# martinResearch/PySparseLP

Measured on AMD Instinct MI355X. Metric: admm_iterations_per_sec, higher is better.
Workload: dtype f64

## Files before the change

include/slp_hip_ext.h:

```cpp
#ifndef SLP_HIP_EXT_H
#define SLP_HIP_EXT_H

#include <stdint.h>

#include "slp_hip.h"
#include "slp_hip_ext_admm_batch.h"
#include "slp_hip_ext_dga_batch.h"

#ifdef __cplusplus
extern "C" {
#endif

int slp_cp_batch_set_stop_gap(slp_cp_batch *s, double tol_gap, double tol_feas, int64_t check_every);
int slp_cp_batch_gap_state(slp_cp_batch *s, int64_t *iterations, int32_t *stopped, double *primal, double *bound, double *violation);

#ifdef __cplusplus
}
#endif
#endif
```

pysparselp_amd/_lib.py:

```python
import ctypes
import os

import numpy as np

_HERE = os.path.dirname(os.path.abspath(__file__))
_VARIANT = os.environ.get("SLP_LIB_VARIANT")
LIB_PATH = os.path.join(_HERE, f"libslp_hip_{_VARIANT}.so" if _VARIANT else "libslp_hip.so")

ORDER_AUTO, ORDER_SEQUENTIAL, ORDER_TREE = 0, 1, 2

_lib = None
_device = None

c_i64 = ctypes.c_int64
c_int = ctypes.c_int
c_dbl = ctypes.c_double
c_vp = ctypes.c_void_p

_SIGNATURES = {
    "slp_version": (c_int, []),
    "slp_build_flags": (c_int, []),
    "slp_device_count": (c_int, []),
    "slp_init": (c_int, [c_int]),
    "slp_synchronize": (c_int, []),
    "slp_trim": (c_int, []),
    "slp_cached_bytes": (c_i64, []),
    "slp_alloc_stats": (c_int, [c_vp, c_int]),
    "slp_last_error": (ctypes.c_char_p, []),
    "slp_timer_start": (c_int, []),
    "slp_timer_stop": (c_int, [c_vp]),
    "slp_matrix_create": (c_vp, [c_i64, c_i64, c_vp, c_vp, c_vp]),
    "slp_matrix_create_stacked": (c_vp, [c_i64, c_i64, c_vp, c_vp, c_vp, c_i64, c_vp, c_vp, c_vp]),
    "slp_matrix_destroy": (None, [c_vp]),
    "slp_matrix_nnz": (c_i64, [c_vp]),
    "slp_matrix_spmv": (c_int, [c_vp, c_vp, c_vp, c_int]),
    "slp_matrix_spmv_t": (c_int, [c_vp, c_vp, c_vp, c_int]),
    "slp_matrix_spmv_abs_pow": (c_int, [c_vp, c_int, c_dbl, c_vp, c_vp]),
    "slp_matrix_spmv2": (c_int, [c_vp, c_int, c_vp, c_vp, c_vp, c_vp]),
    "slp_matrix_download": (c_int, [c_vp, c_int, c_vp, c_vp, c_vp]),
    "slp_matrix_download_rows": (c_int, [c_vp, c_int, c_i64, c_i64, c_vp, c_vp, c_vp]),
    "slp_matrix_bench_spmv": (c_int, [c_vp, c_int, c_int, c_int, c_vp]),
    "slp_product_timing": (c_int, [c_int]),
    "slp_product_timing_read": (c_int, [c_vp]),
    "slp_matrix_gather_rows": (c_vp, [c_vp, c_i64, c_vp, c_vp]),
    "slp_matrix_spmv_kernel": (c_int, [c_vp, c_int]),
    "slp_matrix_set_format": (c_int, [c_vp, c_int]),
    "slp_matrix_release_csr": (c_int, [c_vp]),
    "slp_device_memory": (c_int, [c_vp, c_vp]),
    "slp_matrix_normal": (c_vp, [c_vp, c_dbl, c_dbl]),
    "slp_matrix_remove_columns": (c_vp, [c_vp, c_vp, c_vp, c_vp]),
    "slp_matrix_format_bytes": (c_i64, [c_vp, c_int]),
    "slp_matrix_chunked_create": (c_vp, [c_i64]),
    "slp_matrix_chunked_append": (c_int, [c_vp, c_vp]),
    "slp_matrix_chunks": (c_i64, [c_vp]),
    "slp_matrix_product_launches": (c_i64, [c_vp, c_int]),
    "slp_matrix_strip_width": (c_i64, [c_vp, c_int]),
    "slp_matrix_tall_rows": (c_i64, [c_vp, c_int]),
    "slp_matrix_chunked_expect": (c_int, [c_vp, c_i64]),
    "slp_matrix_chunked_expect_rows": (c_int, [c_vp, c_i64, c_i64]),
    "slp_cp_create": (c_vp, [c_i64, c_i64, c_i64, c_vp, c_vp, c_vp, c_vp, c_vp, c_vp, c_vp, c_vp, c_dbl, c_dbl, c_int]),
    "slp_cp_create_on": (c_vp, [c_vp, c_i64, c_vp, c_vp, c_vp, c_vp, c_vp, c_dbl, c_dbl, c_int]),
    "slp_cp_destroy": (None, [c_vp]),
    "slp_cp_iterate": (c_int, [c_vp, c_i64]),
    "slp_cp_primal_step": (c_int, [c_vp]),
    "slp_cp_split_form": (c_int, [c_vp]),
    "slp_cp_dual_step": (c_int, [c_vp]),
    "slp_cp_report": (c_int, [c_vp, c_vp]),
    "slp_cp_get_x": (c_int, [c_vp, c_vp]),
    "slp_cp_get_y": (c_int, [c_vp, c_vp]),
    "slp_cp_get_preconditioners": (c_int, [c_vp, c_vp, c_vp]),
    "slp_cp_bench": (c_int, [c_vp, c_i64, c_vp]),
    "slp_cp_batch_create": (c_vp, [c_i64, c_i64, c_i64, c_vp, c_vp, c_vp, c_i64, c_vp, c_int, c_vp, c_vp, c_int, c_vp, c_int, c_vp, c_int,
                                   c_dbl, c_dbl]),
    "slp_cp_batch_destroy": (None, [c_vp]),
    "slp_cp_batch_iterate": (c_int, [c_vp, c_i64]),
    "slp_cp_batch_primal_step": (c_int, [c_vp]),
    "slp_cp_batch_dual_step": (c_int, [c_vp]),
    "slp_cp_batch_report": (c_int, [c_vp, c_vp]),
    "slp_cp_batch_get_x": (c_int, [c_vp, c_vp]),
    "slp_cp_batch_get_y": (c_int, [c_vp, c_vp]),
    "slp_cp_batch_get_preconditioners": (c_int, [c_vp, c_vp, c_vp]),
    "slp_cp_batch_bench": (c_int, [c_vp, c_i64, c_vp]),
    "slp_cp_many_create": (c_vp, [c_i64, c_vp, c_vp, c_vp, c_vp, c_vp, c_vp, c_vp, c_vp, c_vp, c_vp, c_vp, c_dbl, c_dbl]),
    "slp_cp_many_destroy": (None, [c_vp]),
    "slp_cp_many_iterate": (c_int, [c_vp, c_i64]),
    "slp_cp_many_primal_step": (c_int, [c_vp]),
    "slp_cp_many_dual_step": (c_int, [c_vp]),
    "slp_cp_many_report": (c_int, [c_vp, c_vp]),
    "slp_cp_many_get_x": (c_int, [c_vp, c_vp]),
    "slp_cp_many_get_y": (c_int, [c_vp, c_vp]),
    "slp_cp_many_get_preconditioners": (c_int, [c_vp, c_vp, c_vp]),
    "slp_cp_many_form": (c_int, [c_vp, c_i64]),
    "slp_cp_many_lds_limit": (c_i64, []),
    "slp_cp_many_bench": (c_int, [c_vp, c_i64, c_vp]),
    "slp_many_cp_set_stop": (c_int, [c_vp, c_dbl, c_i64]),
    "slp_many_cp_stop_state": (c_int, [c_vp, c_vp, c_vp, c_vp]),
    "slp_many_cpgap_set_stop": (c_int, [c_vp, c_dbl, c_dbl, c_i64]),
    "slp_many_cpgap_state": (c_int, [c_vp] * 6),
    "slp_gs_create": (c_vp, [c_i64, c_vp, c_vp, c_vp]),
    "slp_gs_destroy": (None, [c_vp]),
    "slp_gs_num_levels": (c_i64, [c_vp]),
    "slp_gs_sweep_kind": (c_int, [c_vp]),
    "slp_gs_num_bands": (c_int, [c_vp]),
    "slp_gs_solve": (c_int, [c_vp, c_vp, c_vp, c_vp, c_vp, c_int, c_dbl]),
    "slp_admm_create": (c_vp, [c_i64, c_i64, c_vp, c_vp, c_vp, c_vp, c_vp, c_vp, c_vp, c_vp, c_vp, c_vp, c_vp, c_dbl, c_dbl, c_int]),
    "slp_admm_create_lp": (c_vp, [c_i64, c_i64, c_vp, c_vp, c_vp, c_vp, c_i64, c_vp, c_vp, c_vp, c_vp, c_vp, c_vp, c_vp, c_vp, c_vp, c_dbl, c_dbl,
                                  c_int, c_int]),
    "slp_matrix_precondition_rows": (c_vp, [c_vp, c_vp, c_vp]),
    "slp_matrix_standard_form": (c_vp, [c_vp, c_vp]),
    "slp_admm_destroy": (None, [c_vp]),
    "slp_admm_set_xstep": (c_int, [c_vp, c_int]),
    "slp_admm_iterate": (c_int, [c_vp, c_i64]),
    "slp_admm_sweep_step": (c_int, [c_vp]),
    "slp_admm_multiplier_step": (c_int, [c_vp]),
    "slp_admm_report": (c_int, [c_vp, c_vp]),
    "slp_admm_get_x": (c_int, [c_vp, c_vp, c_i64]),
    "slp_admm_get_lambda": (c_int, [c_vp, c_vp]),
    "slp_admm_num_levels": (c_i64, [c_vp]),
    "slp_admm_num_bands": (c_int, [c_vp]),
    "slp_admm_bench": (c_int, [c_vp, c_i64, c_vp]),
    "slp_admm_batch_create_lp": (c_vp, [c_i64, c_i64, c_vp, c_vp, c_vp, c_vp, c_i64, c_vp, c_vp, c_vp, c_vp, c_vp, c_i64, c_vp, c_int, c_vp, c_int,
                                        c_vp, c_int, c_vp, c_int, c_dbl, c_dbl, c_int]),
    "slp_admm_batch_destroy": (None, [c_vp]),
    "slp_admm_batch_iterate": (c_int, [c_vp, c_i64]),
    "slp_admm_batch_sweep_step": (c_int, [c_vp]),
    "slp_admm_batch_multiplier_step": (c_int, [c_vp]),
    "slp_admm_batch_report": (c_int, [c_vp, c_vp]),
    "slp_admm_batch_get_x": (c_int, [c_vp, c_vp, c_i64]),
    "slp_admm_batch_get_lambda": (c_int, [c_vp, c_vp]),
    "slp_admm_batch_num_levels": (c_i64, [c_vp]),
    "slp_admm_batch_form": (c_int, [c_vp]),
    "slp_admm_batch_bench": (c_int, [c_vp, c_i64, c_vp]),
    "slp_admm_many_create": (c_vp, [c_i64, c_vp, c_vp, c_vp, c_vp, c_vp, c_vp, c_vp, c_vp, c_vp, c_vp, c_vp, c_vp, c_vp, c_vp, c_vp, c_vp,
                                    c_dbl, c_dbl, c_int]),
    "slp_admm_many_destroy": (None, [c_vp]),
    "slp_admm_many_iterate": (c_int, [c_vp, c_i64]),
    "slp_admm_many_sweep_step": (c_int, [c_vp]),
    "slp_admm_many_multiplier_step": (c_int, [c_vp]),
    "slp_admm_many_report": (c_int, [c_vp, c_vp]),
    "slp_admm_many_get_x": (c_int, [c_vp, c_vp, c_int]),
    "slp_admm_many_get_lambda": (c_int, [c_vp, c_vp]),
    "slp_admm_many_num_levels": (c_i64, [c_vp, c_i64]),
    "slp_admm_many_form": (c_int, [c_vp, c_i64]),
    "slp_admm_many_lds_limit": (c_i64, []),
    "slp_admm_many_kmax": (c_i64, [c_vp, c_int]),
    "slp_admm_many_bench": (c_int, [c_vp, c_i64, c_vp]),
    "slp_many_admm_set_stop": (c_int, [c_vp, c_dbl, c_dbl, c_i64]),
    "slp_many_admm_stop_state": (c_int, [c_vp, c_vp, c_vp, c_vp, c_vp]),
    "slp_admm_cg_create": (c_vp, [c_i64, c_i64, c_vp, c_vp, c_vp, c_vp, c_vp, c_vp, c_vp, c_vp, c_dbl, c_dbl, c_int]),
    "slp_admm_cg_create_on": (c_vp, [c_vp, c_vp, c_vp, c_vp, c_vp, c_dbl, c_dbl, c_int]),
    "slp_admm_cg_create_on_mixed": (c_vp, [c_vp, c_i64, c_vp, c_vp, c_vp, c_vp, c_dbl, c_dbl, c_int]),
    "slp_blocks_create": (c_vp, [c_i64, c_i64, c_i64, c_vp, c_vp, c_vp, c_vp, c_vp, c_vp, c_vp, c_vp, c_vp, c_vp, c_vp, c_dbl]),
    "slp_blocks_create_on": (c_vp, [c_vp, c_i64, c_vp, c_vp, c_vp, c_vp, c_vp, c_dbl]),
    "slp_blocks_group_link": (c_int, [c_vp, c_int]),
    "slp_blocks_group_iterate": (c_int, [c_vp, c_int, c_i64]),
    "slp_blocks_destroy": (None, [c_vp]),
    "slp_blocks_projection_residual": (c_int, [c_vp, c_vp]),
    "slp_blocks_set_cg": (c_int, [c_vp, c_dbl, c_int]),
    "slp_blocks_set_precond": (c_int, [c_vp, c_int]),
    "slp_blocks_iterate": (c_int, [c_vp, c_i64]),
    "slp_blocks_report": (c_int, [c_vp, c_vp]),
    "slp_blocks_cg_steps": (c_i64, [c_vp]),
    "slp_blocks_get_xp": (c_int, [c_vp, c_vp, c_i64]),
    "slp_admm2_create_on": (c_vp, [c_vp, c_i64, c_vp, c_vp, c_vp, c_vp, c_vp, c_vp, c_dbl]),
    "slp_admm2_destroy": (None, [c_vp]),
    "slp_admm2_set_cg": (c_int, [c_vp, c_dbl, c_int]),
    "slp_admm2_iterate": (c_int, [c_vp, c_i64]),
    "slp_admm2_report": (c_int, [c_vp, c_vp]),
    "slp_admm2_cg_steps": (c_i64, [c_vp]),
    "slp_admm2_get_x": (c_int, [c_vp, c_vp, c_i64]),
    "slp_admm2_projection_residual": (c_int, [c_vp, c_vp]),
    "slp_dga_create_on": (c_vp, [c_vp, c_i64, c_vp, c_vp, c_vp, c_vp, c_vp]),
    "slp_dga_destroy": (None, [c_vp]),
    "slp_dga_set_path": (c_int, [c_vp, c_int]),
    "slp_dga_path": (c_int, [c_vp]),
    "slp_dga_iterate": (c_int, [c_vp, c_i64]),
    "slp_dga_iterations": (c_i64, [c_vp]),
    "slp_dga_push_random": (c_int, [c_vp, c_vp, c_i64]),
    "slp_dga_status": (c_int, [c_vp, c_vp]),
    "slp_dga_get_x": (c_int, [c_vp, c_vp]),
    "slp_dga_get_y": (c_int, [c_vp, c_vp]),
    "slp_dga_report": (c_int, [c_vp, c_vp]),
    "slp_dga_timing": (c_int, [c_vp, c_int]),
    "slp_dga_timing_read": (c_int, [c_vp, c_vp]),
    "slp_dga_line_search": (c_int, [c_vp, c_vp, c_vp, c_vp, c_vp, c_vp, c_int, c_vp, c_i64, c_vp]),
    "slp_batch_dga_create_on": (c_vp, [c_vp, c_i64, c_vp, c_i64, c_vp, c_vp, c_int, c_vp, c_int, c_vp, c_int]),
    "slp_batch_dga_destroy": (None, [c_vp]),
    "slp_batch_dga_set_path": (c_int, [c_vp, c_int]),
    "slp_batch_dga_path": (c_int, [c_vp]),
    "slp_batch_dga_sort": (c_int, [c_vp]),
    "slp_batch_dga_iterate": (c_int, [c_vp, c_i64]),
    "slp_batch_dga_iterations": (c_i64, [c_vp]),
    "slp_batch_dga_push_random": (c_int, [c_vp, c_vp, c_i64]),
    "slp_batch_dga_status": (c_int, [c_vp, c_vp]),
    "slp_batch_dga_frozen": (c_int, [c_vp, c_vp]),
    "slp_batch_dga_get_x": (c_int, [c_vp, c_vp]),
    "slp_batch_dga_get_y": (c_int, [c_vp, c_vp]),
    "slp_batch_dga_report": (c_int, [c_vp, c_vp]),
    "slp_batch_dga_timing": (c_int, [c_vp, c_int]),
    "slp_batch_dga_timing_read": (c_int, [c_vp, c_vp]),
    "slp_many_dga_create": (c_vp, [c_i64, c_vp, c_vp, c_vp, c_vp, c_vp, c_vp, c_vp, c_vp, c_vp, c_vp, c_vp, c_vp]),
    "slp_many_dga_destroy": (None, [c_vp]),
    "slp_many_dga_iterate": (c_int, [c_vp, c_i64]),
    "slp_many_dga_push_random": (c_int, [c_vp, c_vp, c_i64]),
    "slp_many_dga_status": (c_int, [c_vp, c_vp]),
    "slp_many_dga_frozen": (c_int, [c_vp, c_vp]),
    "slp_many_dga_get_x": (c_int, [c_vp, c_vp]),
    "slp_many_dga_get_y": (c_int, [c_vp, c_vp]),
    "slp_many_dga_report": (c_int, [c_vp, c_vp]),
    "slp_many_dga_timing": (c_int, [c_vp, c_int]),
    "slp_many_dga_timing_read": (c_int, [c_vp, c_vp]),
    "slp_many_dga_kmax": (c_i64, [c_vp]),
    "slp_many_dual_set_stop": (c_int, [c_vp, c_dbl, c_i64]),
    "slp_many_dual_stop_state": (c_int, [c_vp, c_vp, c_vp, c_vp]),
    "slp_admm_cg_create_on_two_sided": (c_vp, [c_vp, c_i64, c_vp, c_vp, c_vp, c_vp, c_vp, c_dbl, c_dbl, c_int]),
    "slp_admm_cg_create_on_lp": (c_vp, [c_vp, c_i64, c_vp, c_vp, c_vp, c_vp, c_vp, c_vp, c_dbl, c_dbl, c_int, c_int]),
    "slp_admm_cg_create_lp": (c_vp, [c_i64, c_i64, c_vp, c_vp, c_vp, c_vp, c_i64, c_vp, c_vp, c_vp, c_vp, c_vp, c_vp, c_vp, c_vp, c_vp,
                                     c_dbl, c_dbl, c_int, c_int]),
    "slp_admm_cg_destroy": (None, [c_vp]),
    "slp_admm_cg_set_reuse": (c_int, [c_vp, c_int]),
    "slp_admm_cg_iterate": (c_int, [c_vp, c_i64]),
    "slp_admm_cg_xstep": (c_int, [c_vp]),
    "slp_admm_cg_multiplier_step": (c_int, [c_vp]),
    "slp_admm_cg_report": (c_int, [c_vp, c_vp]),
    "slp_admm_cg_get_x": (c_int, [c_vp, c_vp, c_i64]),
    "slp_matrix_random": (c_vp, [c_i64, c_i64, c_dbl, ctypes.c_uint64, c_i64]),
    "slp_random_lp_vectors": (c_int, [c_vp, c_dbl, ctypes.c_uint64, c_i64, c_vp, c_vp, c_vp, c_vp, c_vp]),
    "slp_random_lp_vectors_eq": (c_int, [c_vp, c_dbl, ctypes.c_uint64, c_i64, c_i64, c_vp, c_vp, c_vp, c_vp, c_vp]),
    "slp_comm_unique_id": (c_int, [c_vp]),
    "slp_comm_init": (c_int, [c_int, c_int, c_vp]),
    "slp_comm_init_host": (c_int, [c_int, c_int, c_vp, c_vp]),
    "slp_comm_finalize": (c_int, []),
    "slp_comm_allreduce_host": (c_int, [c_vp, c_i64, c_int]),
    "slp_comm_barrier": (c_int, []),
    "slp_comm_bench_allreduce": (c_int, [c_i64, c_int, c_vp]),
    "slp_comm_info": (c_int, [c_vp, c_vp]),
    "slp_comm_collectives": (ctypes.c_longlong, []),
    "slp_comm_timing": (c_int, [c_int]),
    "slp_comm_timing_read": (c_int, [c_vp]),
}

EXPORTED_SYMBOLS = tuple(_SIGNATURES)

_EXT_SIGNATURES = {
    "slp_cp_batch_set_stop_gap": (c_int, [c_vp, c_dbl, c_dbl, c_i64]),
    "slp_cp_batch_gap_state": (c_int, [c_vp] * 6),
}

EXT_SYMBOLS = tuple(_EXT_SIGNATURES)

_EXT_ADMM_BATCH_SIGNATURES = {
    "slp_admm_batch_set_stop": (c_int, [c_vp, c_dbl, c_dbl, c_i64]),
    "slp_admm_batch_stop_state": (c_int, [c_vp] * 5),
}

EXT_ADMM_BATCH_SYMBOLS = tuple(_EXT_ADMM_BATCH_SIGNATURES)

_EXT_DGA_BATCH_SIGNATURES = {
    "slp_batch_dga_set_stop": (c_int, [c_vp, c_dbl, c_vp, c_i64]),
    "slp_batch_dga_stop_state": (c_int, [c_vp] * 5),
}

EXT_DGA_BATCH_SYMBOLS = tuple(_EXT_DGA_BATCH_SIGNATURES)

HOST_ALLREDUCE_FN = ctypes.CFUNCTYPE(c_int, ctypes.POINTER(c_dbl), c_i64, c_int, c_vp)


class SlpError(RuntimeError):
    """Raised for every failure reported by libslp_hip.so (and when it is absent)."""


def load():
    global _lib
    if _lib is not None:
        return _lib
    if not os.path.exists(LIB_PATH):
        raise SlpError(
            f"{LIB_PATH} is missing: build it with `python -c 'import __graft_entry__ as g; g.build()'` "
            "or `make -C pysparselp_amd/csrc`.  pysparselp_amd has no CPU fallback."
        )
    try:
        lib = ctypes.CDLL(LIB_PATH, mode=ctypes.RTLD_GLOBAL)
    except OSError as e:
        raise SlpError(f"cannot load {LIB_PATH}: {e}") from e
    for name, (res, args) in (list(_SIGNATURES.items()) + list(_EXT_SIGNATURES.items()) + list(_EXT_ADMM_BATCH_SIGNATURES.items())
                              + list(_EXT_DGA_BATCH_SIGNATURES.items())):
        fn = getattr(lib, name)
        fn.restype = res
        fn.argtypes = args
    flags = int(lib.slp_build_flags())
    if flags and not _VARIANT:
        raise SlpError(f"{LIB_PATH} is a kernel-lab build (slp_build_flags() = {flags}: bit 0 = -DSLP_ABLATION kernels with parts removed, "
                       "WRONG results; bit 1 = `make variant`): it is only loaded when SLP_LIB_VARIANT names it.  Rebuild with "
                       "`make -C pysparselp_amd/csrc clean all`.")
    _lib = lib
    return lib


def last_error():
    msg = load().slp_last_error()
    return msg.decode("utf-8", "replace") if msg else "unknown error"


def check(rc):
    if rc != 0:
        raise SlpError(last_error())


def check_handle(h):
    if not h:
        raise SlpError(last_error())
    return h


def lib(device=None):
    global _device
    l = load()
    if _device is None:
        dev = device
        if dev is None:
            dev = int(os.environ.get("SLP_DEVICE", os.environ.get("LOCAL_RANK", "0")))
            n = l.slp_device_count()
            if n > 0 and dev >= n:
                raise SlpError(f"device index {dev} (SLP_DEVICE / LOCAL_RANK) but only {n} HIP device(s) are visible")
        check(l.slp_init(int(dev)))
        _device = int(dev)
    elif device is not None and int(device) != _device:
        raise SlpError(f"process already bound to device {_device}")
    return l


def ptr(a):
    if a is None:
        return None
    assert a.flags.c_contiguous
    return a.ctypes.data_as(c_vp)


def f64(a):
    return np.ascontiguousarray(a, dtype=np.float64)


def csr_arrays(a):
    return (np.ascontiguousarray(a.indptr, dtype=np.int64), np.ascontiguousarray(a.indices, dtype=np.int32),
            np.ascontiguousarray(a.data, dtype=np.float64))
```

pysparselp_amd/csrc/slp_chunked.hip:

```cpp
#include "slp_common.h"
#include "slp_kernels.h"

slp_matrix::~slp_matrix() {
    for (slp_matrix *c : chunks) delete c;
}

namespace slp {

void composite_of_chunks(const slp_matrix *g, bool transposed, size_t k0, size_t k1, StripJds &f) {
    f.parts.clear();
    f.part_off.clear();
    f.parts_cols = transposed;
    f.ok = k1 > k0;
    f.nrow = transposed ? g->a.ncol : g->a.nrow;
    f.ncol = transposed ? g->a.nrow : g->a.ncol;
    f.nnz = 0;
    f.D = 0;
    f.tall = true;
    bool first = true;
    for (size_t k = k0; k < k1; ++k) {
        const StripJds *p = transposed ? &g->chunks[k]->fat : &g->chunks[k]->fa;
        f.parts.push_back(p);
        f.part_off.push_back(g->chunk_row0[k]);
        f.nnz += g->chunks[k]->a.nnz;
        f.D = first ? p->D : (p->D > 0 && f.D > 0 ? std::max(f.D, p->D) : 0);
        f.tall = f.tall && p->tall;
        first = false;
    }
    f.fused = f.tall && tall_fuse(f);
}

static void refresh_composites(slp_matrix *g) {
    for (int t = 0; t < 2; ++t) composite_of_chunks(g, t != 0, 0, g->chunks.size(), t ? g->fat : g->fa);
    g->at.nrow = g->a.ncol;
    g->at.ncol = g->a.nrow;
    g->at.nnz = g->a.nnz;
}

}

using namespace slp;

extern "C" {

slp_matrix *slp_matrix_chunked_create(int64_t ncol) {
    SLP_API_PTR({
        SLP_REQUIRE(ncol > 0 && ncol < ((i64)1 << 31), "slp_matrix_chunked_create: bad column count");
        ctx();
        auto *g = new slp_matrix();
        g->a.ncol = ncol;
        g->tried_fa = g->tried_fat = true;
        g->have_at = true;
        g->csr_released = true;
        return g;
    })
}

int slp_matrix_chunked_append(slp_matrix *g, slp_matrix *c) {
    SLP_API_INT({
        SLP_REQUIRE(g && c && g != c, "slp_matrix_chunked_append: NULL argument");
        SLP_REQUIRE(g->csr_released && g->a.ptr.p == nullptr && (g->a.nrow == 0 || !g->chunks.empty()),
                    "slp_matrix_chunked_append: the first argument is not a chunked matrix (slp_matrix_chunked_create)");
        SLP_REQUIRE(c->chunks.empty() && !c->csr_released, "slp_matrix_chunked_append: the chunk must be a plain matrix with its CSR");
        SLP_REQUIRE(c->a.ncol == g->a.ncol, "slp_matrix_chunked_append: the chunk has another column count");
        SLP_REQUIRE(c->a.nrow > 0 && c->a.nnz > 0, "slp_matrix_chunked_append: empty chunk");
        SLP_REQUIRE(g->borrowers == 0, "slp_matrix_chunked_append: a solver created on the chunked matrix is alive");
        SLP_REQUIRE(c->borrowers == 0 && !c->scaled, "slp_matrix_chunked_append: the chunk is in use by a solver (or was scaled in place)");
        SLP_REQUIRE(g->a.nrow % 2 == 0, "slp_matrix_chunked_append: every chunk but the last must have an even number of rows");
        Phase ph("slp_matrix_chunked_append");
        if (g->expect_rows > 0 && g->a.nrow + c->a.nrow <= g->expect_rows && !c->tried_fa) {
            const char *e = getenv("SLP_TALL_FUSE");
            if (!(e && e[0] == '0')) {
                c->tall_rows_before = g->a.nrow;
                c->tall_rows_total = g->expect_rows;
            }
        } else if (g->expect_chunks > 1 && !c->tried_fa) {
            const char *e = getenv("SLP_TALL_FUSE");
            if (!(e && e[0] == '0')) {
                i64 a = ctx().num_cu, b = g->expect_chunks;
                while (b) { const i64 t = a % b; a = b; b = t; }
                c->tall_block_multiple = ctx().num_cu / a;
            }
        }
        if (!c->tried_fa && !c->tried_fat)
            for (int t = 0; t < 2; ++t) c->tall_carry[t] = g->tall_carry[t];
        const StripJds *f0 = fast_format(c, false), *f1 = fast_format(c, true);
        SLP_REQUIRE(f0 && f1, "slp_matrix_chunked_append: the chunk does not qualify for strip copies in both orientations (too small or "
                              "unsorted rows): use an ordinary matrix for problems of that size");
        if (f0->D > 0 && f1->D > 0) {
            c->rowsq.alloc(2 * (size_t)c->a.nrow);
            matrix_row_squares(c->a, c->rowsq.p);
        }
        if (g->chunks.empty())
            for (int t = 0; t < 2; ++t) {
                const StripJds *f = t ? f1 : f0;
                if (f->tall && f->S == 1) {
                    g->tall_carry[t].C = f->C; g->tall_carry[t].dcap = f->D > 0 ? f->tall_dcap : -1;
                    g->tall_carry[t].R = f->tall_R; g->tall_carry[t].total = f->tall_total;
                }
            }
        if (f0->tall) g->tall_carry[0].blocks += f0->B;
        SLP_REQUIRE(slp_matrix_release_csr(c) == 0, slp_last_error());
        c->a.ptr.release();
        c->at.ptr.release();
        g->chunks.push_back(c);
        g->chunk_row0.push_back(g->a.nrow);
        g->a.nrow += c->a.nrow;
        g->a.nnz += c->a.nnz;
        g->a.max_row_len = std::max(g->a.max_row_len, c->a.max_row_len);
        refresh_composites(g);
        if ((i64)g->chunks.size() < g->expect_chunks) {
            std::vector<size_t> sizes;
            for (const StripJds *f : {f0, f1})
                if (f->tall)
                    for (const auto &b : f->tall_pay) sizes.push_back(b.cap);
            dev_reserve_async(sizes);
        }
    })
}

int slp_matrix_chunked_expect(slp_matrix *g, int64_t chunks) {
    SLP_API_INT({
        SLP_REQUIRE(g && g->csr_released && g->a.ptr.p == nullptr && chunks >= 0, "slp_matrix_chunked_expect: bad arguments");
        g->expect_chunks = chunks;
    })
}

int slp_matrix_chunked_expect_rows(slp_matrix *g, int64_t chunks, int64_t rows) {
    SLP_API_INT({
        SLP_REQUIRE(g && g->csr_released && g->a.ptr.p == nullptr && chunks >= 0 && rows >= 0, "slp_matrix_chunked_expect_rows: bad arguments");
        g->expect_chunks = chunks;
        g->expect_rows = rows;
    })
}

int64_t slp_matrix_chunks(const slp_matrix *g) { return g ? (int64_t)g->chunks.size() : -1; }

int64_t slp_matrix_strip_width(slp_matrix *m, int transposed) {
    if (!m) return -1;
    int64_t c = 0;
    const int rc = [&]() -> int {
        SLP_API_INT({
            const StripJds *f = fast_format(m, transposed != 0);
            if (f && !m->chunks.empty() && !f->parts.empty()) f = f->parts[0];
            c = (f && f->ok) ? (int64_t)f->C : 0;
        })
    }();
    return rc == 0 ? c : -1;
}

int64_t slp_matrix_tall_rows(slp_matrix *m, int transposed) {
    if (!m) return -1;
    int64_t r = 0;
    const int rc = [&]() -> int {
        SLP_API_INT({
            const StripJds *f = fast_format(m, transposed != 0);
            if (f && !m->chunks.empty() && !f->parts.empty()) f = f->parts[0];
            r = (f && f->ok && f->tall) ? (int64_t)f->tall_R : 0;
        })
    }();
    return rc == 0 ? r : -1;
}

int64_t slp_matrix_product_launches(const slp_matrix *g, int transposed) {
    if (!g) return -1;
    if (g->chunks.empty()) return 1;
    return (transposed ? g->fat : g->fa).fused ? 1 : (int64_t)g->chunks.size();
}

}
```

pysparselp_amd/csrc/slp_common.h:

```cpp
#pragma once
#include <hip/hip_runtime.h>

#include <cstdint>
#include <cstdio>
#include <cstdlib>
#include <cstring>
#include <mutex>
#include <stdexcept>
#include <string>
#include <vector>

#include "../../include/slp_hip.h"
#include "slp_tall_plan.h"

#if !defined(SLP_ABLATION) && (defined(SLP_TALL_ABL) || defined(SLP_GS_ABLATE) || defined(SLP_GS_BANDS_ABLATE_FETCH) || \
                               defined(SLP_GS_BANDS_ABLATE_PUBLISH) || defined(SLP_GS_BANDS_ABLATE_SC1) || defined(SLP_STRIP_ABLATE))
#error "a kernel-lab macro (SLP_TALL_ABL / SLP_GS_ABLATE / SLP_GS_BANDS_ABLATE_* / SLP_STRIP_ABLATE) without -DSLP_ABLATION: ablated kernels give wrong results and must not be built into libslp_hip.so"
#endif

namespace slp {

typedef int64_t i64;
typedef int32_t i32;

void set_error(const std::string &msg);

struct Error : std::runtime_error {
    using std::runtime_error::runtime_error;
};

#define SLP_HIP(expr)                                                                     \
    do {                                                                                  \
        hipError_t e_ = (expr);                                                           \
        if (e_ != hipSuccess)                                                             \
            throw slp::Error(std::string(#expr) + " failed: " + hipGetErrorString(e_) +   \
                             " (" __FILE__ ":" + std::to_string(__LINE__) + ")");         \
    } while (0)

#define SLP_REQUIRE(cond, msg)                       \
    do {                                             \
        if (!(cond)) throw slp::Error(std::string(msg)); \
    } while (0)

#define SLP_API_INT(...)                   \
    try {                                  \
        __VA_ARGS__;                       \
        return 0;                          \
    } catch (const std::exception &e) {    \
        slp::set_error(e.what());          \
        return 1;                          \
    }

#define SLP_API_PTR(...)                   \
    try {                                  \
        __VA_ARGS__;                       \
    } catch (const std::exception &e) {    \
        slp::set_error(e.what());          \
        return nullptr;                    \
    }

struct Context {
    bool ready = false;
    int device = -1;
    int num_cu = 256;
    hipStream_t stream = nullptr;
    hipEvent_t ev0 = nullptr, ev1 = nullptr;
};
Context &ctx();
Context &ctx_unchecked();

bool trace_enabled();
double trace_now();
void trace_slow(const char *what, size_t bytes, double t0);

void *dev_alloc(size_t bytes, size_t *capacity);
void dev_free(void *p, size_t capacity);
void dev_reserve_async(const std::vector<size_t> &sizes);

template <class T>
struct DevBuf {
    T *p = nullptr;
    size_t n = 0;
    size_t cap = 0;
    DevBuf() = default;
    explicit DevBuf(size_t count) { alloc(count); }
    DevBuf(const DevBuf &) = delete;
    DevBuf &operator=(const DevBuf &) = delete;
    DevBuf(DevBuf &&o) noexcept : p(o.p), n(o.n), cap(o.cap) { o.p = nullptr; o.n = 0; o.cap = 0; }
    DevBuf &operator=(DevBuf &&o) noexcept {
        if (this != &o) { release(); p = o.p; n = o.n; cap = o.cap; o.p = nullptr; o.n = 0; o.cap = 0; }
        return *this;
    }
    ~DevBuf() { release(); }
    void release() {
        if (p) dev_free(p, cap);
        p = nullptr;
        n = 0;
        cap = 0;
    }
    void alloc(size_t count) {
        release();
        p = static_cast<T *>(dev_alloc((count ? count : 1) * sizeof(T), &cap));
        n = count;
    }
    void upload(const T *host, size_t count) {
        if (count > n || !p) alloc(count);
        if (count) SLP_HIP(hipMemcpyAsync(p, host, count * sizeof(T), hipMemcpyHostToDevice, ctx().stream));
        SLP_HIP(hipStreamSynchronize(ctx().stream));
    }
    void download(T *host, size_t count) const {
        if (count) SLP_HIP(hipMemcpyAsync(host, p, count * sizeof(T), hipMemcpyDeviceToHost, ctx().stream));
        SLP_HIP(hipStreamSynchronize(ctx().stream));
    }
    void zero() {
        if (n) SLP_HIP(hipMemsetAsync(p, 0, n * sizeof(T), ctx().stream));
    }
    void copy_from(const DevBuf<T> &o) {
        if (o.n > n || !p) alloc(o.n);
        if (o.n) SLP_HIP(hipMemcpyAsync(p, o.p, o.n * sizeof(T), hipMemcpyDeviceToDevice, ctx().stream));
    }
};

inline std::mutex &capture_mutex() {
    static std::mutex m;
    return m;
}

struct IterGraph {
    hipGraph_t graph = nullptr;
    hipGraphExec_t exec = nullptr;
    int unroll = 0;
    ~IterGraph() { reset(); }
    void reset() {
        if (exec) (void)hipGraphExecDestroy(exec);
        if (graph) (void)hipGraphDestroy(graph);
        exec = nullptr;
        graph = nullptr;
        unroll = 0;
    }
    template <class F>
    void run(i64 k, int want_unroll, F body) {
        hipStream_t st = ctx().stream;
        if (want_unroll > k) want_unroll = (int)k;
        const char *off = getenv("SLP_NO_GRAPH");
        if (!exec && k >= 2 && want_unroll >= 1 && !(off && off[0] == '1')) {
            std::lock_guard<std::mutex> no_helper_calls(capture_mutex());
            SLP_HIP(hipStreamBeginCapture(st, hipStreamCaptureModeThreadLocal));
            try {
                for (int u = 0; u < want_unroll; ++u) body();
            } catch (...) {
                hipGraph_t dead = nullptr;
                (void)hipStreamEndCapture(st, &dead);
                if (dead) (void)hipGraphDestroy(dead);
                throw;
            }
            SLP_HIP(hipStreamEndCapture(st, &graph));
            SLP_HIP(hipGraphInstantiate(&exec, graph, nullptr, nullptr, 0));
            unroll = want_unroll;
        }
        if (exec) {
            for (; k >= unroll; k -= unroll) SLP_HIP(hipGraphLaunch(exec, st));
        }
        for (; k > 0; --k) body();
    }
};

struct Phase {
    const char *name;
    double t0 = 0.0;
    bool on;
    static bool enabled() { return trace_enabled(); }
    static double now() { return trace_now(); }
    explicit Phase(const char *n) : name(n), on(enabled()) {
        if (on) { (void)hipStreamSynchronize(ctx().stream); t0 = now(); }
    }
    ~Phase() {
        if (on) { (void)hipStreamSynchronize(ctx().stream); fprintf(stderr, "[slp trace] %-34s %9.3f ms\n", name, (now() - t0) * 1e3); }
    }
};

inline int grid_for(i64 work_items, int block, int max_blocks_per_cu = 8) {
    i64 g = (work_items + block - 1) / block;
    i64 cap = (i64)ctx().num_cu * max_blocks_per_cu;
    if (g > cap) g = cap;
    if (g < 1) g = 1;
    return (int)g;
}

struct CsrDev {
    i64 nrow = 0, ncol = 0, nnz = 0;
    DevBuf<i64> ptr;
    DevBuf<i32> idx;
    DevBuf<double> val;
    i64 max_row_len = 0;
    double mean_row_len() const { return nrow ? (double)nnz / (double)nrow : 0.0; }
};

struct TallWg {
    const unsigned int *dir;
    const unsigned int *pay;
    const double *val;
    const double *dict;
    i64 npk;
    i64 row0;
    i64 x0;
    i64 ncol;
    int nrows;
    int D;
};

struct StripJds {
    bool ok = false;
    i64 nrow = 0, ncol = 0, nnz = 0, T = 0, B = 0;
    int S = 1;
    DevBuf<double> part;
    mutable DevBuf<double> part2;
    DevBuf<i64> base;
    DevBuf<unsigned short> perm;
    DevBuf<unsigned char> slen;
    DevBuf<unsigned int> soff;
    DevBuf<double> val;
    DevBuf<unsigned short> col;
    int C = 0;
    int D = 0;
    bool wide = false;
    int rpl = 2;
    DevBuf<unsigned short> ent;
    const double *dict = nullptr;
    bool tall = false;
    int tall_R = 0;
    int tall_dcap = 0;
    i64 tall_total = 0;
    DevBuf<TallWg> tall_wg;
    std::vector<DevBuf<unsigned int>> tall_dir;
    std::vector<DevBuf<unsigned int>> tall_pay;
    std::vector<DevBuf<double>> tall_val;
    size_t tall_bytes = 0;
    std::vector<const StripJds *> parts;
    std::vector<i64> part_off;
    bool parts_cols = false;
    bool fused = false;
};
struct ValueDict {
    int state = -1;
    int D = 0;
    DevBuf<double> values;
    DevBuf<unsigned long long> keys;
};
bool value_dictionary(const CsrDev &a, ValueDict &d);
bool strip_wanted(const CsrDev &a, int variant);
bool strip_build(const CsrDev &a, StripJds &f, const ValueDict *dict, int variant);
void strip_spmv(const StripJds &f, const double *x, double *out);
void product_timing(bool on);
void product_timing_read(double out[3]);
extern int g_strip_single_chain;
bool strip_has_tall_split(const StripJds &f);
void strip_spmv2(const StripJds &f, const double *x0, const double *x1, double *out0, double *out1);
void strip_spmv_with_dict(const StripJds &f, const double *table, const double *x, double *out);
void strip_spmv_pow(const StripJds &f, double pw, const double *x, double *out);
bool strip_abs_pow_supported(const StripJds &f);
void strip_spmv_abs_pow(const StripJds &f, double pw, const double *x, double *out);
bool tall_wanted(i64 nrow, i64 ncol, i64 nnz);
struct TallCarry {
    int C = 0, dcap = -1, R = 0;
    i64 total = 0;
    i64 blocks = 0;
};
bool tall_build(const CsrDev &a, bool transposed, StripJds &f, const ValueDict *dict, i64 block_multiple = 0, i64 rows_before = 0,
                i64 rows_total = 0, const TallCarry *carry = nullptr);
void tall_spmv(const StripJds &f, const double *x, double *out, int accum);
bool tall_fuse(StripJds &composite);
void tall_spmv_fused(const StripJds &composite, const double *x, double *out);
void tall_spmv_pow(const StripJds &f, double pw, const double *x, double *out, int accum);
size_t strip_format_bytes(const StripJds &f);

}

struct slp_matrix {
    slp::CsrDev a;
    slp::CsrDev at;
    bool have_at = false;
    slp::StripJds fa, fat;
    bool tried_fa = false, tried_fat = false;
    slp::ValueDict vdict;
    slp::DevBuf<double> vx, vy;
    int format_policy = 0;
    bool scaled = false;
    int borrowers = 0;
    int csr_bound = 0;
    bool csr_released = false;
    std::vector<slp_matrix *> chunks;
    std::vector<slp::i64> chunk_row0;
    slp::DevBuf<double> rowsq;
    slp::i64 expect_chunks = 0;
    slp::i64 tall_block_multiple = 0;
    slp::i64 tall_rows_before = 0, tall_rows_total = 0;
    slp::i64 expect_rows = 0;
    slp::TallCarry tall_carry[2];
    ~slp_matrix();
};

namespace slp {
void finish_stats(CsrDev &a);
void build_transpose(slp_matrix *m);
void ensure_transposed(slp_matrix *m);
void matrix_row_squares(const CsrDev &a, double *sq);
int lanes_for(const CsrDev &a, int order);
void launch_spmv(const CsrDev &a, const double *x, double *y, int order);
const StripJds *fast_format(slp_matrix *m, bool transposed);
void matrix_spmv(slp_matrix *m, bool transposed, const double *x, double *y, int order);
slp_matrix *matrix_precondition_rows(slp_matrix *a, double *b, double *b2);
slp_matrix *matrix_standard_form(slp_matrix *a_eq, slp_matrix *a_ineq);
void invalidate_derived(slp_matrix *m);
void require_csr(const slp_matrix *m, const char *what);
bool matrix_dictionary(slp_matrix *m);
slp_matrix *matrix_row_slice(slp_matrix *m, i64 r0, i64 r1);
void matrix_drop_csr(slp_matrix *m);
void composite_of_chunks(const slp_matrix *g, bool transposed, size_t k0, size_t k1, StripJds &f);
}
```

pysparselp_amd/csrc/slp_tall.hip:

```cpp
#include <atomic>
#include <cmath>
#include <cstdlib>
#include <cstring>
#include <vector>

#include <rocprim/rocprim.hpp>

#include "slp_common.h"
#include "slp_kernels.h"
#include "slp_tall.h"

namespace slp {


__global__ void k_tall_range(i64 nrow, const i64 *__restrict__ ptr, const i32 *__restrict__ idx, i64 c0, i64 c1,
                             i64 *__restrict__ lo, i64 *__restrict__ len) {
    for (i64 r = (i64)blockIdx.x * blockDim.x + threadIdx.x; r < nrow; r += (i64)gridDim.x * blockDim.x) {
        const i64 s = ptr[r], e = ptr[r + 1];
        auto lower = [&](i64 c) {
            i64 a = s, b = e;
            while (a < b) {
                const i64 mid = (a + b) >> 1;
                if ((i64)idx[mid] < c) a = mid + 1;
                else b = mid;
            }
            return a;
        };
        const i64 l = lower(c0), h = lower(c1);
        lo[r] = l;
        len[r] = h - l;
    }
    if (blockIdx.x == 0 && threadIdx.x == 0) len[nrow] = 0;
}

__global__ __launch_bounds__(kBlock) void k_tall_sorted(i64 nnz, const i32 *__restrict__ idx, i64 nrow, const i64 *__restrict__ ptr,
                                                        int *__restrict__ bad) {
    const int lane = threadIdx.x & (kWave - 1);
    const i64 wave = ((i64)blockIdx.x * kBlock + threadIdx.x) / kWave, nwaves = (i64)gridDim.x * kBlock / kWave;
    for (i64 r = wave; r < nrow; r += nwaves) {
        const i64 s = ptr[r], e = ptr[r + 1];
        for (i64 k = s + 1 + lane; k < e; k += kWave)
            if (idx[k - 1] >= idx[k]) atomicOr(bad, 1);
    }
    (void)nnz;
}

template <bool TR>
__global__ __launch_bounds__(kBlock) void k_tall_keys(i64 r0, i64 nrow, int R, i64 T, int C, i64 b0, int D, const unsigned long long *__restrict__ dkeys,
                                                      const i64 *__restrict__ ptr, const i32 *__restrict__ idx,
                                                      const double *__restrict__ val, const i64 *__restrict__ lo,
                                                      const i64 *__restrict__ opos, i64 obase, unsigned long long *__restrict__ keys,
                                                      double *__restrict__ kvals, int *__restrict__ bad) {
    __shared__ unsigned long long skey[kTallDictMax];
    for (int q = threadIdx.x; q < D; q += kBlock) skey[q] = dkeys[q];
    __syncthreads();
    const int lane = threadIdx.x & (kWave - 1);
    const i64 wave = ((i64)blockIdx.x * kBlock + threadIdx.x) / kWave, nwaves = (i64)gridDim.x * kBlock / kWave;
    for (i64 rr = wave; rr < nrow; rr += nwaves) {
        const i64 r = r0 + rr;
        const i64 s = TR ? lo[rr] : ptr[r];
        const i64 e = TR ? s + (opos[rr + 1] - opos[rr]) : ptr[r + 1];
        const i64 o = TR ? opos[rr] : s - obase;
        for (i64 k = s + lane; k < e; k += kWave) {
            const i32 j = idx[k];
            if (!TR && k > s && idx[k - 1] >= j) atomicOr(bad, 1);
            int id = 0;
            if (D > 0) {
                const unsigned long long key = tall_value_key((unsigned long long)__double_as_longlong(val[k]));
                int hi = D - 1;
                while (id < hi) {
                    const int mid = (id + hi) >> 1;
                    if (skey[mid] < key) id = mid + 1;
                    else hi = mid;
                }
                if (skey[id] != key) atomicOr(bad, 2);
            }
            const i64 trow = TR ? (i64)j : r, tcol = TR ? r : (i64)j;
            const unsigned long long b = (unsigned long long)(trow / R - b0), rl = (unsigned long long)(trow % R);
            const unsigned int ts = (unsigned int)tcol / (unsigned int)C;
            const unsigned long long t = ts, cl = (unsigned int)tcol - ts * (unsigned int)C;
            keys[o + (k - s)] = ((b * (unsigned long long)T + t) << kTallCellShift) | (rl << (kTallIdBits + kTallColBits)) | (cl << kTallIdBits) |
                                (unsigned long long)id;
            if (kvals) kvals[o + (k - s)] = val[k];
        }
    }
}

__global__ void k_tall_cellptr(i64 nnz, i64 ncell, const unsigned long long *__restrict__ key, i64 *__restrict__ cptr) {
    for (i64 p = (i64)blockIdx.x * blockDim.x + threadIdx.x; p < nnz; p += (i64)gridDim.x * blockDim.x) {
        const i64 c = (i64)(key[p] >> kTallCellShift), prev = p > 0 ? (i64)(key[p - 1] >> kTallCellShift) : -1;
        for (i64 j = prev + 1; j <= c; ++j) cptr[j] = p;
        if (p == nnz - 1)
            for (i64 j = c + 1; j <= ncell; ++j) cptr[j] = nnz;
    }
}

#define SLP_OPAQUE(v) asm volatile("" : "+v"(v))
template <int CTRL, int ROWS = 0xf>
__device__ __forceinline__ unsigned int tall_dpp(unsigned int x) {
    return (unsigned int)__builtin_amdgcn_update_dpp(0, (int)x, CTRL, ROWS, 0xf, true);
}
template <int CTRL, int ROWS = 0xf>
__device__ __forceinline__ unsigned long long tall_dpp(unsigned long long x) {
    return (unsigned long long)tall_dpp<CTRL, ROWS>((unsigned int)(x >> 32)) << 32 | tall_dpp<CTRL, ROWS>((unsigned int)x);
}
template <int SEG, typename U>
__device__ __forceinline__ U tall_lane_sums(U x) {
    x += tall_dpp<0x111>(x);
    x += tall_dpp<0x112>(x);
    x += tall_dpp<0x114>(x);
    x += tall_dpp<0x118>(x);
    x += tall_dpp<0x142, 0xa>(x);
    if (SEG == 64) x += tall_dpp<0x143, 0xc>(x);
    return x;
}
__device__ __forceinline__ unsigned long long tall_block_scan(unsigned long long v, unsigned long long *wtot, unsigned long long *tot) {
    int lane = threadIdx.x & (kWave - 1), w = threadIdx.x / kWave;
    SLP_OPAQUE(w);
    const unsigned long long inc = tall_lane_sums<kWave>(v);
    if (lane == kWave - 1) wtot[w] = inc;
    __syncthreads();
    unsigned long long base = 0, all = 0;
    for (int i = 0; i < kTallT / kWave; ++i) {
        const unsigned long long t = wtot[i];
        if (i < w) base += t;
        all += t;
    }
    __syncthreads();
    *tot = all;
    return base + inc - v;
}

#define SLP_TB_PROF(k) do {} while (0)
struct TallScan {
    unsigned long long *w;
    unsigned long long *p;
    unsigned long long *before_w, *before_p;
    unsigned long long *ticket;
};
constexpr unsigned long long kScanMask = (1ull << 62) - 1;
__device__ __forceinline__ void tall_scan_put(const TallScan &sc, i64 c, unsigned long long level, unsigned long long w, unsigned long long k) {
    __hip_atomic_store(&sc.w[c], (level << 62) | w, __ATOMIC_RELAXED, __HIP_MEMORY_SCOPE_AGENT);
    __hip_atomic_store(&sc.p[c], (level << 62) | k, __ATOMIC_RELAXED, __HIP_MEMORY_SCOPE_AGENT);
}
__device__ __forceinline__ unsigned int tall_scan_get(const TallScan &sc, i64 c, unsigned long long *w, unsigned long long *k) {
    for (;;) {
        const unsigned long long a = __hip_atomic_load(&sc.w[c], __ATOMIC_RELAXED, __HIP_MEMORY_SCOPE_AGENT);
        const unsigned long long b = __hip_atomic_load(&sc.p[c], __ATOMIC_RELAXED, __HIP_MEMORY_SCOPE_AGENT);
        if (!(a >> 62) || (a >> 62) != (b >> 62)) continue;
        *w = a & kScanMask;
        *k = b & kScanMask;
        return (unsigned int)(a >> 62);
    }
}

__device__ __forceinline__ i64 tall_range_of(i64 t, i64 T, int S) {
    i64 s = t * S / T;
    while (T * (s + 1) / S <= t) ++s;
    while (T * s / S > t) --s;
    return s;
}

template <bool DICT>
__global__ __launch_bounds__(kTallT) void k_tall_build(int R, i64 T, int S, int C, unsigned int sum0, i64 ncell, const unsigned long long *__restrict__ keys,
                                                       const double *__restrict__ svals, const i64 *__restrict__ cellptr, TallScan sc,
                                                       i64 cap_w, i64 cap_p, TallPkt *__restrict__ sdir,
                                                       unsigned int *__restrict__ spay, double *__restrict__ spayv) {
    __shared__ unsigned int cnt[kTallRmax];
    __shared__ unsigned int rstart[kTallRmax];
    __shared__ unsigned short posrow[kTallRmax];
    __shared__ unsigned int nlane[kTallT];
    __shared__ unsigned long long wtot[kTallT / kWave];
    __shared__ unsigned int width[kTallSlots];
    __shared__ unsigned int bcnt[kTallBuckets * 32], bstart[kTallBuckets * 32 + 1];
    __shared__ unsigned long long cbuf[2 * 32 * 33], ctot[2 * 32];
    __shared__ unsigned int ccls[32 * 33], call[32];
    __shared__ unsigned int spare1x[33];
    __shared__ unsigned int lackx[(kTallBuckets - 1) * 32], sparex[(kTallBuckets - 1) * 33];
    __shared__ i64 s_cell, s_c0, s_tn;
    __shared__ int s_n;
    __shared__ unsigned int s_dump[kWave];
    __shared__ unsigned long long s_before_w, s_before_p;
    static_assert(sizeof(cnt) + sizeof(rstart) + sizeof(posrow) == (size_t)kTallBuildRowBytes * kTallRmax, "tall cells: builder LDS per row");
    static_assert(sizeof(nlane) + sizeof(wtot) + sizeof(width) + sizeof(bcnt) + sizeof(bstart) + sizeof(cbuf) + sizeof(ctot) + sizeof(ccls) + sizeof(call) +
                          sizeof(spare1x) + sizeof(lackx) + sizeof(sparex) + 3 * sizeof(i64) + sizeof(int) + sizeof(s_dump) + 2 * sizeof(unsigned long long) + 128 <=
                      (size_t)kTallBuildFixed,
                  "tall cells: builder LDS (128 bytes for the alignment of its parts)");
    auto tile_of = [&](i64 t) -> unsigned int { return t >= 0 ? (unsigned int)(t * C) : kNoTile; };
    auto take_next = [&](unsigned long long drawn) {
        i64 c = (i64)drawn, lo = 0, hi = 0, hi2 = 0;
        for (;;) {
            if (c >= ncell) break;
            lo = cellptr[c];
            hi = cellptr[c + 1];
            hi2 = cellptr[c + 1 < ncell ? c + 2 : c + 1];
            if (hi > lo) break;
            tall_scan_put(sc, c, 1ull, 0ull, 0ull);
            c = (i64)atomicAdd(sc.ticket, 1ull);
        }
        s_cell = c;
        if (c < ncell) {
            const i64 b = c / T, t = c % T;
            const i64 t_end = S > 1 ? T * (tall_range_of(t, T, S) + 1) / S : T;
            i64 tn = -1;
            if (t + 1 < t_end && hi2 > hi) tn = t + 1;
            else
                for (i64 u = t + 2; u < t_end; ++u)
                    if (cellptr[b * T + u + 1] > cellptr[b * T + u]) { tn = u; break; }
            s_tn = tn;
            s_c0 = lo;
            s_n = (int)(hi - lo);
        }
    };
    static_assert(kTallT >= 2 * kWave, "take_next runs on the first lane of the second wave, beside wave 0's look-back");
    if (threadIdx.x == kWave) take_next(atomicAdd(sc.ticket, 1ull));
    for (;;) {
        int p = threadIdx.x;
        SLP_OPAQUE(p);
        __syncthreads();
        SLP_TB_PROF(0);
        const i64 cell = s_cell;
        if (cell >= ncell) break;
        const i64 t = cell % T, tn = s_tn, c0 = s_c0;
        const int n = s_n;
        unsigned long long drawn = 0;
        for (int r = p; r < R; r += kTallT) cnt[r] = 0;
        __syncthreads();
        SLP_TB_PROF(1);
        for (int i0 = p; i0 < n; i0 += 4 * kTallT) {
            unsigned long long ka[4], kb[4];
#pragma unroll
            for (int j = 0; j < 4; ++j) {
                const int i = i0 + j * kTallT < n ? i0 + j * kTallT : n - 1;
                ka[j] = keys[c0 + i];
                kb[j] = keys[c0 + (i > 0 ? i - 1 : 0)];
            }
#pragma unroll
            for (int j = 0; j < 4; ++j) {
                const int i = i0 + j * kTallT;
                if (i < n) {
                    const unsigned int r = (unsigned int)(ka[j] >> (kTallIdBits + kTallColBits)) & ((1u << kTallRowBits) - 1);
                    const unsigned int rp = i > 0 ? (unsigned int)(kb[j] >> (kTallIdBits + kTallColBits)) & ((1u << kTallRowBits) - 1) : ~0u;
                    if (r != rp) rstart[r] = (unsigned int)i;
                    atomicAdd(&cnt[r], 1u);
                }
            }
        }
        __syncthreads();
        SLP_TB_PROF(2);
        const int crows = R > (int)(p & 31) ? (R - (int)(p & 31) + 31) / 32 : 0;
        const int mpl = ((R + 31) / 32 + 31) / 32;
        const int m0 = (p >> 5) * mpl < crows ? (p >> 5) * mpl : crows, m1 = m0 + mpl < crows ? m0 + mpl : crows;
        auto class_scan2 = [&](unsigned long long *v, unsigned long long *tot) {
            const int mine = 2 * ((p & 31) * 33 + (p >> 5)), theirs = 2 * ((p >> 5) * 33 + (p & 31));
            cbuf[mine] = v[0];
            cbuf[mine + 1] = v[1];
            __syncthreads();
            const unsigned long long u0 = cbuf[theirs], u1 = cbuf[theirs + 1];
            const unsigned long long s0 = tall_lane_sums<32>(u0), s1 = tall_lane_sums<32>(u1);
            cbuf[theirs] = s0 - u0;
            cbuf[theirs + 1] = s1 - u1;
            if ((p & 31) == 31) { ctot[2 * (p >> 5)] = s0; ctot[2 * (p >> 5) + 1] = s1; }
            __syncthreads();
            v[0] = cbuf[mine];
            v[1] = cbuf[mine + 1];
            tot[0] = ctot[2 * (p & 31)];
            tot[1] = ctot[2 * (p & 31) + 1];
        };
        unsigned long long ha = 0, hb = 0;
        for (int m = m0; m < m1; ++m) {
            const unsigned int c = cnt[(p & 31) + 32 * m];
            if (c) {
                const unsigned int cl = c < (unsigned)kTallBuckets ? c : kTallBuckets;
                if (cl > 3) ha += 1ull << (21 * (kTallBuckets - cl));
                else hb += 1ull << (21 * (3 - cl));
            }
        }
        unsigned long long hv[2] = {ha, hb}, tv[2];
        class_scan2(hv, tv);
        unsigned long long ea = hv[0], eb = hv[1];
        const unsigned long long ta = tv[0], tb = tv[1];
        if (p < 32)
            for (int cl = kTallBuckets; cl >= 1; --cl)
                bcnt[(kTallBuckets - cl) * 32 + p] = (unsigned int)(((cl > 3 ? ta : tb) >> (21 * ((cl > 3 ? kTallBuckets : 3) - cl))) & 0x1fffffu);
        __syncthreads();
        SLP_TB_PROF(3);
        if (p < kWave) {
            const unsigned int c0 = bcnt[3 * p], c1 = bcnt[3 * p + 1], c2 = bcnt[3 * p + 2];
            unsigned int inc = c0 + c1 + c2;
#pragma unroll
            for (int off = 1; off < kWave; off <<= 1) {
                const unsigned int o = __shfl_up(inc, off, kWave);
                if (p >= off) inc += o;
            }
            const unsigned int ex = inc - (c0 + c1 + c2);
            bstart[3 * p] = ex;
            bstart[3 * p + 1] = ex + c0;
            bstart[3 * p + 2] = ex + c0 + c1;
            if (p == kWave - 1) bstart[kTallBuckets * 32] = inc;
        }
        __syncthreads();
        SLP_TB_PROF(4);
        if (p < (kTallBuckets - 1) * 32) {
            const unsigned int k = (unsigned)p >> 5, r = (unsigned)p & 31u;
            const unsigned int S = bstart[k * 32], E = bstart[k * 32 + 32];
            const unsigned int first = S + ((r + 32u - (S & 31u)) & 31u), nl = first < E ? (E - first + 31u) / 32u : 0u;
            const unsigned int rr = bstart[k * 32 + r + 1] - bstart[k * 32 + r];
            const unsigned int lack = nl > rr ? nl - rr : 0u, spare = rr > nl ? rr - nl : 0u;
            const unsigned int il = tall_lane_sums<32>(lack), is = tall_lane_sums<32>(spare);
            lackx[k * 32 + r] = il - lack;
            sparex[k * 33 + r] = is - spare;
            if (r == 31u) sparex[k * 33 + 32] = is;
        }
        for (int m = m0; m < m1; ++m) {
            const unsigned int r = (unsigned int)((p & 31) + 32 * m), c = cnt[r];
            if (c) {
                const unsigned int cl = c < (unsigned)kTallBuckets ? c : kTallBuckets;
                unsigned int within;
                if (cl > 3) { within = (unsigned int)((ea >> (21 * (kTallBuckets - cl))) & 0x1fffffu); ea += 1ull << (21 * (kTallBuckets - cl)); }
                else { within = (unsigned int)((eb >> (21 * (3 - cl))) & 0x1fffffu); eb += 1ull << (21 * (3 - cl)); }
                posrow[bstart[(kTallBuckets - cl) * 32 + (p & 31)] + within] = (unsigned short)r;
            }
        }
        __syncthreads();
        SLP_TB_PROF(5);
        const unsigned int npos = bstart[kTallBuckets * 32];
        const unsigned int n2 = bstart[(kTallBuckets - 1) * 32];
        const bool fill = n2 <= (unsigned)kTallT;
        const unsigned int rho = (unsigned)p & 31u;
        unsigned int pos0 = npos, c0p = 0;
        if (fill) {
            if ((unsigned)p < n2) {
                int cl = kTallBuckets;
                while (cl > 2 && (unsigned)p >= bstart[(kTallBuckets - cl + 1) * 32]) --cl;
                const unsigned int *bs = bstart + (kTallBuckets - cl) * 32;
                const unsigned int S = bs[0], E = bs[32];
                auto lanes_of = [&](unsigned int r) -> unsigned int {
                    const unsigned int first = S + ((r + 32u - (S & 31u)) & 31u);
                    return first < E ? (E - first + 31u) / 32u : 0u;
                };
                const unsigned int first = S + ((rho + 32u - (S & 31u)) & 31u), i = ((unsigned)p - first) / 32u;
                const unsigned int nr = bs[rho + 1] - bs[rho];
                if (i < nr) {
                    pos0 = bs[rho] + i;
                } else {
                    const unsigned int k = (unsigned)(kTallBuckets - cl);
                    const unsigned int u = i - nr + lackx[k * 32 + rho];
                    const unsigned int *sx = sparex + k * 33;
                    if (u < sx[32]) {
                        unsigned int lo = 0, hi = 32;
#pragma unroll
                        for (int it = 0; it < 5; ++it) { const unsigned int mid = (lo + hi) >> 1; if (sx[mid] <= u) lo = mid; else hi = mid; }
                        pos0 = bs[lo] + lanes_of(lo) + (u - sx[lo]);
                    }
                }
                c0p = cnt[posrow[pos0]];
            }
        } else {
            pos0 = (unsigned)p < npos ? (unsigned)p : npos;
            c0p = pos0 < npos ? cnt[posrow[pos0]] : 0u;
        }
        unsigned int mine = c0p, own0 = 0, nown = 0, left0 = 0, nleft = 0;
        {
            const unsigned int *b1 = bstart + (kTallBuckets - 1) * 32;
            const unsigned int tau = (unsigned)n / kTallT + ((unsigned)p < (unsigned)n % kTallT ? 1u : 0u);
            const unsigned int want = (fill && c0p < tau) ? tau - c0p : 0u;
            ccls[rho * 33 + (p >> 5)] = want;
            __syncthreads();
            {
                const int theirs = (p >> 5) * 33 + (int)rho;
                const unsigned int u = ccls[theirs], su = tall_lane_sums<32>(u);
                ccls[theirs] = su - u;
                if (rho == 31u) call[p >> 5] = su;
            }
            __syncthreads();
            const unsigned int before = ccls[rho * 33 + (p >> 5)], all = call[rho];
            const unsigned int n1 = b1[rho + 1] - b1[rho];
            own0 = b1[rho] + before;
            nown = before >= n1 ? 0u : (want < n1 - before ? want : n1 - before);
            if (p < 32) {
                const unsigned int sp = n1 > all ? n1 - all : 0u;
                const unsigned int is = tall_lane_sums<32>(sp);
                spare1x[p] = is - sp;
                if (p == 31) spare1x[32] = is;
            }
            __syncthreads();
            SLP_TB_PROF(6);
            if (p == kWave) drawn = atomicAdd(sc.ticket, 1ull);
            unsigned long long total;
            left0 = (unsigned int)tall_block_scan(want - nown, wtot, &total);
            const unsigned int nspare = spare1x[32];
            nleft = left0 >= nspare ? 0u : (want - nown < nspare - left0 ? want - nown : nspare - left0);
            if (fill) mine += nown + nleft;
            else for (unsigned int pos = p + kTallT; pos < npos; pos += kTallT) mine += cnt[posrow[pos]];
        }
        auto rowpos = [&](unsigned int q) -> unsigned int {
            if (!fill) { const unsigned int pos = q * kTallT + p; return pos < npos ? pos : npos; }
            if (pos0 < npos) { if (q == 0) return pos0; --q; }
            if (q < nown) return own0 + q;
            q -= nown;
            if (q >= nleft) return npos;
            const unsigned int *b1 = bstart + (kTallBuckets - 1) * 32;
            const unsigned int u = left0 + q;
            unsigned int lo = 0, hi = 32;
#pragma unroll
            for (int it = 0; it < 5; ++it) { const unsigned int mid = (lo + hi) >> 1; if (spare1x[mid] <= u) lo = mid; else hi = mid; }
            return b1[lo + 1] - (spare1x[lo + 1] - spare1x[lo]) + (u - spare1x[lo]);
        };
        unsigned int cover = mine;
        {
            const int lane = p & (kWave - 1), w = p / kWave;
#pragma unroll
            for (int off = 1; off < kWave; off <<= 1) {
                const unsigned int o = __shfl_down(cover, off, kWave);
                if (lane + off < kWave) cover = o > cover ? o : cover;
            }
            if (lane == 0) wtot[w] = cover;
            __syncthreads();
            unsigned int right = 0;
            for (int i = w + 1; i < kTallT / kWave; ++i) right = (unsigned int)wtot[i] > right ? (unsigned int)wtot[i] : right;
            cover = right > cover ? right : cover;
            __syncthreads();
        }
        nlane[p] = cover;
        unsigned long long cw = 0;
        {
            unsigned long long w = cover;
            if (DICT) w += (cover + 7u) / 8u + (cover > 4u ? (cover - 4u + 7u) / 8u : 0u);
            w = tall_lane_sums<kWave>(w);
            if ((p & (kWave - 1)) == kWave - 1) wtot[p / kWave] = w;
        }
        __syncthreads();
        SLP_TB_PROF(7);
        const unsigned int longest = nlane[0];
        const unsigned int nxt = p + 1 < kTallT ? nlane[p + 1] : 0u;
        for (int i = 0; i < kTallT / kWave; ++i) cw += wtot[i];
        const unsigned long long cell_w = (cw + 3ull) & ~3ull, cell_p = longest ? (longest + kTallSlots - 1) / kTallSlots : 1u;
        if (p == 0) tall_scan_put(sc, cell, 1ull, cell_w, cell_p);
        bool fits = true;
        unsigned int *pay = nullptr;
        double *payv = nullptr;
        TallPkt *pk = nullptr;
        unsigned int woff = 0, npk = 0;
        unsigned int q = 0, s = 0, mypos = rowpos(0);
        unsigned int myrow = mypos < npos ? posrow[mypos] : 0u, mycnt = mypos < npos ? cnt[myrow] : 0u;
        for (unsigned int g = 0; g * kTallSlots < longest || g == 0; ++g) {
#pragma unroll
            for (int j = 0; j < kTallSlots; ++j) {
                const unsigned int k = g * kTallSlots + j;
                if (nxt <= k && k < cover) width[j] = (unsigned int)p + 1u;
                if (p == 0 && cover <= k) width[j] = 0u;
            }
            __syncthreads();
            SLP_TB_PROF(8);
            unsigned int wd[kTallSlots], words = 0;
            for (int j = 0; j < kTallSlots; ++j) { wd[j] = width[j]; words += wd[j]; }
            const unsigned int hi0 = words, hi1 = words + wd[0];
            if (DICT) words += wd[0] + wd[4];
            unsigned int kofs[kTallSlots], have = 0;
#pragma unroll
            for (int j = 0; j < kTallSlots; ++j) {
                kofs[j] = 0;
                if ((unsigned)p < wd[j] && mypos < npos) {
                    kofs[j] = rstart[myrow] + s;
                    have |= 1u << j;
                    if (++s == mycnt) {
                        ++q; s = 0;
                        mypos = rowpos(q);
                        myrow = mypos < npos ? posrow[mypos] : 0u;
                        mycnt = mypos < npos ? cnt[myrow] : 0u;
                    }
                }
            }
            unsigned long long key[kTallSlots];
            double value[kTallSlots];
#pragma unroll
            for (int j = 0; j < kTallSlots; ++j) {
                key[j] = (have >> j & 1u) ? keys[c0 + kofs[j]] : 0ull;
                value[j] = (!DICT && (have >> j & 1u)) ? svals[c0 + kofs[j]] : 0.0;
            }
            if (g == 0) {
                if (p == kWave) take_next(drawn);
                if (p < kWave) {
                    unsigned long long bw = 0, bp = 0;
                    for (i64 j = cell - 1; j >= 0; j -= kWave) {
                        const i64 qc = j - p;
                        unsigned int st = 2u;
                        unsigned long long w = 0, k = 0;
                        if (qc >= 0) st = tall_scan_get(sc, qc, &w, &k);
                        const unsigned long long summed = __ballot(st == 2u);
                        const int f = summed ? __ffsll((long long)summed) - 1 : kWave;
                        if (p > f) { w = 0; k = 0; }
#pragma unroll
                        for (int off = kWave / 2; off; off >>= 1) { w += __shfl_xor(w, off, kWave); k += __shfl_xor(k, off, kWave); }
                        bw += w; bp += k;
                        if (summed) break;
                    }
                    if (p == 0) {
                        tall_scan_put(sc, cell, 2ull, bw + cell_w, bp + cell_p);
                        sc.before_w[cell] = bw;
                        sc.before_p[cell] = bp;
                        s_before_w = bw;
                        s_before_p = bp;
                    }
                }
                __syncthreads();
                SLP_TB_PROF(9);
                if (s_cell < ncell && p * 16 < s_n) {
                    const unsigned int *g = reinterpret_cast<const unsigned int *>(keys + s_c0) + p * 32;
                    const unsigned int lds = __builtin_amdgcn_readfirstlane((unsigned int)(size_t)s_dump);
                    unsigned int m0_saved;
                    asm volatile("s_mov_b32 %0, m0\n\ts_mov_b32 m0, %1\n\ts_nop 0\n\tglobal_load_lds_dword %2, off\n\ts_mov_b32 m0, %0"
                                 : "=&s"(m0_saved) : "s"(lds), "v"(g) : "memory");
                }
                fits = (i64)(s_before_w + cell_w) <= cap_w && (i64)(s_before_p + cell_p) <= cap_p;
                pay = spay + s_before_w;
                payv = DICT ? nullptr : spayv + s_before_w;
                pk = sdir + s_before_p;
            }
            if (!fits) break;
            {
                unsigned int *base = pay + woff;
                unsigned int hb0 = 0, hb1 = 0, so = 0;
#pragma unroll
                for (int j = 0; j < kTallSlots; ++j) {
                    if ((unsigned)p < wd[j]) {
                        unsigned int item = 0u, hib = 0u;
                        if (have >> j & 1u) {
                            const unsigned int r1 = ((unsigned int)(key[j] >> (kTallIdBits + kTallColBits)) & ((1u << kTallRowBits) - 1)) + sum0;
                            const unsigned int cl = (unsigned int)(key[j] >> kTallIdBits) & (kTallC - 1);
                            if (DICT) {
                                const TallItem it = tall_item_encode((unsigned int)key[j] & ((1u << kTallIdBits) - 1), cl, r1);
                                item = it.word;
                                hib = it.fifth;
                            } else {
                                item = tall_item64_encode(cl, r1);
                            }
                        }
                        base[so + p] = item;
                        if (!DICT) payv[woff + so + p] = value[j];
                        if (j < 4) hb0 |= hib << (8 * j);
                        else hb1 |= hib << (8 * (j - 4));
                    }
                    so += wd[j];
                }
                if (DICT && (unsigned)p < wd[0]) base[hi0 + p] = hb0;
                if (DICT && (unsigned)p < wd[4]) base[hi1 + p] = hb1;
                if (p == 0) {
                    TallPkt h;
                    h.off = woff;
                    h.xsrc = (g == 0) ? (kPktNewCell | tile_of(tn)) : kNoTile;
                    for (int i = 0; i < 4; ++i) h.c[i] = wd[2 * i] | (wd[2 * i + 1] << 16);
                    h.strip = (unsigned int)t;
                    h.pad = 0;
                    pk[npk] = h;
                }
            }
            woff += words;
            ++npk;
            __syncthreads();
            SLP_TB_PROF(10);
        }
    }
}

template <bool DICT>
__global__ __launch_bounds__(kBlock) void k_tall_estimate(i64 ncell, const i64 *__restrict__ cellptr, unsigned long long *__restrict__ est) {
    unsigned long long w = 0, k = 0;
    for (i64 c = (i64)blockIdx.x * kBlock + threadIdx.x; c < ncell; c += (i64)gridDim.x * kBlock) {
        const unsigned long long n = (unsigned long long)(cellptr[c + 1] - cellptr[c]);
        if (!n) continue;
        const unsigned long long L = n < (unsigned)kTallT ? n : (unsigned)kTallT, tau = (n + kTallT - 1) / kTallT;
        unsigned long long cw = n;
        if (DICT) cw += L * ((tau + 7) / 8 + (tau > 4 ? (tau - 4 + 7) / 8 : 0));
        w += (cw + 3ull) & ~3ull;
        k += (tau + kTallSlots - 1) / kTallSlots;
    }
#pragma unroll
    for (int off = kWave / 2; off; off >>= 1) { w += __shfl_xor(w, off, kWave); k += __shfl_xor(k, off, kWave); }
    if ((threadIdx.x & (kWave - 1)) == 0) { atomicAdd(&est[0], w); atomicAdd(&est[1], k); }
}

__global__ void k_tall_streams(i64 V, i64 T, int S, const i64 *__restrict__ cellptr, TallScan sc, i64 *__restrict__ ext) {
    for (i64 v = (i64)blockIdx.x * blockDim.x + threadIdx.x; v < V; v += (i64)gridDim.x * blockDim.x) {
        const i64 b = v / S, cs = b * T + T * (v % S) / S, ce = b * T + T * (v % S + 1) / S;
        auto before = [&](i64 c, i64 *w, i64 *k) {
            for (--c; c >= 0 && cellptr[c + 1] == cellptr[c];) --c;
            *w = c >= 0 ? (i64)(sc.w[c] & kScanMask) : 0;
            *k = c >= 0 ? (i64)(sc.p[c] & kScanMask) : 0;
        };
        i64 w0, p0, w1, p1;
        before(cs, &w0, &p0);
        before(ce, &w1, &p1);
        ext[4 * v] = w0;
        ext[4 * v + 1] = w1 - w0;
        ext[4 * v + 2] = p0;
        ext[4 * v + 3] = p1 - p0;
    }
}

__global__ void k_tall_dir(i64 ncell, i64 V, i64 T, int S, int C, const i64 *__restrict__ cellptr, TallScan sc, const i64 *__restrict__ ext,
                           const i64 *__restrict__ pkt_ptr, const TallPkt *__restrict__ sdir, TallPkt *__restrict__ dir) {
    const i64 i0 = (i64)blockIdx.x * blockDim.x + threadIdx.x, step = (i64)gridDim.x * blockDim.x;
    for (i64 c = i0; c < ncell; c += step) {
        if (cellptr[c + 1] == cellptr[c]) continue;
        const i64 pk0 = (i64)sc.before_p[c], np = (i64)(sc.p[c] & kScanMask) - pk0, w0 = (i64)sc.before_w[c];
        const i64 b = c / T, t = c % T, v = b * S + (S > 1 ? tall_range_of(t, T, S) : 0);
        TallPkt *out = dir + pkt_ptr[v] + 1 + (pk0 - ext[4 * v + 2]);
        for (i64 j = 0; j < np; ++j) {
            TallPkt h = sdir[pk0 + j];
            h.off += (unsigned int)(w0 - ext[4 * v]);
            out[j] = h;
        }
    }
    for (i64 v = i0; v < V; v += step) {
        const i64 b = v / S, t_begin = T * (v % S) / S, t_end = T * (v % S + 1) / S;
        i64 first = -1;
        for (i64 u = t_begin; u < t_end; ++u)
            if (cellptr[b * T + u + 1] > cellptr[b * T + u]) { first = u; break; }
        TallPkt h;
        h.off = 0; h.xsrc = first >= 0 ? (unsigned int)(first * C) : kNoTile;
        h.c[0] = h.c[1] = h.c[2] = h.c[3] = 0; h.strip = 0; h.pad = 0;
        dir[pkt_ptr[v]] = h;
        h.off = (unsigned int)ext[4 * v + 1];
        h.xsrc = kNoTile;
        for (i64 k = pkt_ptr[v] + 1 + ext[4 * v + 3]; k < pkt_ptr[v + 1]; ++k) dir[k] = h;
    }
}
static int tall_env(const char *name) {
    const char *e = getenv(name);
    return e ? atoi(e) : 0;
}

static i64 tall_pass_nnz() {
    const char *e = getenv("SLP_TALL_PASS_NNZ");
    const i64 v = e ? atoll(e) : 500000000ll;
    return v > 0 ? v : 500000000ll;
}

bool tall_build(const CsrDev &a, bool transposed, StripJds &f, const ValueDict *dict, i64 block_multiple, i64 rows_before, i64 rows_total,
                const TallCarry *carry) {
    Phase ph(transposed ? "tall_build (A^T from the CSR of A)" : "tall_build");
    hipStream_t st = ctx().stream;
    f = StripJds();
    if ((dict && (dict->D <= 0 || dict->D > kTallDictMax)) || a.nrow == 0 || a.ncol == 0 || a.nnz == 0) return false;
    const i64 nrowF = transposed ? a.ncol : a.nrow, ncolF = transposed ? a.nrow : a.ncol;
    if (ncolF * 8 >= ((i64)1 << 31)) return false;
    TallPlanIn pin;
    pin.nrow = nrowF; pin.ncol = ncolF; pin.nnz = a.nnz; pin.D = dict ? dict->D : 0; pin.cus = ctx().num_cu;
    if (!transposed) { pin.block_multiple = block_multiple; pin.rows_before = rows_before; pin.rows_total = rows_total; }
    pin.env_R = std::max(0, tall_env("SLP_TALL_R")); pin.env_C = tall_env("SLP_TALL_C"); pin.env_split = tall_env("SLP_TALL_SPLIT");
    if (carry && carry->C > 0) {
        pin.carry_C = carry->C; pin.carry_dcap = carry->dcap; pin.carry_total = transposed ? 0 : carry->total;
        pin.carry_R = transposed ? carry->R : 0;
        pin.carry_blocks = transposed ? 0 : carry->blocks;
    }
    const TallPlan plan = tall_plan(pin);
    SLP_REQUIRE(plan.lds_bytes <= kTallLdsBytes && plan.build_lds_bytes <= kTallLdsBytes && plan.R >= 1 && plan.R <= kTallRmax,
                "tall_build: the planned geometry does not fit the LDS");
    const int R = plan.R, S = plan.S, Cw = plan.C;
    const i64 T = plan.T;
    const unsigned int sum0 = tall_item_sum_base(plan.dcap);
    SLP_REQUIRE(sum0 + (unsigned int)R <= (1u << kTallRowBits), "tall_build: sum field");
    const i64 B = (nrowF + R - 1) / R, ncell = B * T, V = B * S;
    unsigned int cellbits = 1;
    while (((i64)1 << cellbits) < ncell) ++cellbits;
    if (kTallCellShift + cellbits > 64) return false;
    i64 P = (a.nnz + tall_pass_nnz() - 1) / tall_pass_nnz();
    P = std::max<i64>(1, std::min<i64>(P, B));
    DevBuf<int> bad(1);
    bad.zero();
    if (transposed) {
        hipLaunchKernelGGL(k_tall_sorted, dim3(grid_for(a.nrow * kWave, kBlock)), dim3(kBlock), 0, st, a.nnz, a.idx.p, a.nrow, a.ptr.p, bad.p);
        SLP_HIP(hipGetLastError());
        int hbad = 0;
        bad.download(&hbad, 1);
        if (hbad) return false;
    }
    DevBuf<unsigned long long> sorted((size_t)a.nnz);
    DevBuf<double> svals;
    if (!dict) svals.alloc((size_t)a.nnz);
    {
        Phase p1("  tall: keys + sort");
        DevBuf<i64> lo, len, opos;
        if (transposed) { lo.alloc((size_t)a.nrow); len.alloc((size_t)a.nrow + 1); opos.alloc((size_t)a.nrow + 1); }
        const int D = dict ? dict->D : 0;
        const unsigned long long *dk = dict ? dict->keys.p : (const unsigned long long *)nullptr;
        const unsigned b0 = transposed ? (unsigned)(kTallIdBits + kTallColBits) : (unsigned)kTallCellShift, b1 = (unsigned)kTallCellShift + cellbits;
        i64 done = 0;
        for (i64 pass = 0; pass < P; ++pass) {
            const i64 bb0 = B * pass / P, bb1 = B * (pass + 1) / P;
            if (bb1 == bb0) continue;
            const i64 f0 = bb0 * (i64)R, f1 = std::min<i64>(bb1 * (i64)R, nrowF);
            i64 n_p = 0, obase = 0;
            if (!transposed) {
                i64 ends[2];
                SLP_HIP(hipMemcpyAsync(&ends[0], a.ptr.p + f0, sizeof(i64), hipMemcpyDeviceToHost, st));
                SLP_HIP(hipMemcpyAsync(&ends[1], a.ptr.p + f1, sizeof(i64), hipMemcpyDeviceToHost, st));
                SLP_HIP(hipStreamSynchronize(st));
                obase = ends[0];
                n_p = ends[1] - ends[0];
            } else {
                hipLaunchKernelGGL(k_tall_range, dim3(grid_for(a.nrow, kBlock)), dim3(kBlock), 0, st, a.nrow, a.ptr.p, a.idx.p, f0, f1, lo.p, len.p);
                SLP_HIP(hipGetLastError());
                size_t bytes = 0;
                SLP_HIP(rocprim::exclusive_scan(nullptr, bytes, len.p, opos.p, (i64)0, (size_t)a.nrow + 1, rocprim::plus<i64>(), st));
                DevBuf<char> tmp(bytes);
                SLP_HIP(rocprim::exclusive_scan(tmp.p, bytes, len.p, opos.p, (i64)0, (size_t)a.nrow + 1, rocprim::plus<i64>(), st));
                SLP_HIP(hipMemcpyAsync(&n_p, opos.p + a.nrow, sizeof(i64), hipMemcpyDeviceToHost, st));
                SLP_HIP(hipStreamSynchronize(st));
            }
            if (n_p == 0) continue;
            DevBuf<unsigned long long> keys((size_t)n_p);
            DevBuf<double> kvals;
            if (!dict && transposed) kvals.alloc((size_t)n_p);
            const i64 scan_rows = transposed ? a.nrow : f1 - f0, r0 = transposed ? 0 : f0;
            if (transposed)
                hipLaunchKernelGGL((k_tall_keys<true>), dim3(grid_for(scan_rows * kWave, kBlock)), dim3(kBlock), 0, st, r0, scan_rows, R, T, Cw, (i64)0, D, dk,
                                   a.ptr.p, a.idx.p, a.val.p, lo.p, opos.p, obase, keys.p, kvals.p, bad.p);
            else
                hipLaunchKernelGGL((k_tall_keys<false>), dim3(grid_for(scan_rows * kWave, kBlock)), dim3(kBlock), 0, st, r0, scan_rows, R, T, Cw, (i64)0, D, dk,
                                   a.ptr.p, a.idx.p, a.val.p, (const i64 *)nullptr, (const i64 *)nullptr, obase, keys.p, (double *)nullptr, bad.p);
            SLP_HIP(hipGetLastError());
            size_t bytes = 0;
            if (dict) {
                SLP_HIP(rocprim::radix_sort_keys(nullptr, bytes, keys.p, sorted.p + done, (size_t)n_p, b0, b1, st));
                DevBuf<char> tmp(bytes);
                SLP_HIP(rocprim::radix_sort_keys(tmp.p, bytes, keys.p, sorted.p + done, (size_t)n_p, b0, b1, st));
                SLP_HIP(hipStreamSynchronize(st));
            } else {
                const double *vin = transposed ? kvals.p : a.val.p + obase;
                SLP_HIP(rocprim::radix_sort_pairs(nullptr, bytes, keys.p, sorted.p + done, vin, svals.p + done, (size_t)n_p, b0, b1, st));
                DevBuf<char> tmp(bytes);
                SLP_HIP(rocprim::radix_sort_pairs(tmp.p, bytes, keys.p, sorted.p + done, vin, svals.p + done, (size_t)n_p, b0, b1, st));
                SLP_HIP(hipStreamSynchronize(st));
            }
            done += n_p;
        }
        int hbad = 0;
        bad.download(&hbad, 1);
        if (hbad || done != a.nnz) return false;
    }
    DevBuf<i64> cellptr((size_t)ncell + 1);
    hipLaunchKernelGGL(k_tall_cellptr, dim3(grid_for(a.nnz, kBlock)), dim3(kBlock), 0, st, a.nnz, ncell, sorted.p, cellptr.p);
    SLP_HIP(hipGetLastError());
    Phase p2("  tall: packets (one pass)");
    DevBuf<unsigned long long> scan(4 * (size_t)ncell + 1), est(2);
    TallScan sc;
    sc.w = scan.p; sc.p = scan.p + ncell; sc.ticket = scan.p + 2 * ncell; sc.before_w = sc.ticket + 1; sc.before_p = sc.before_w + ncell;
    est.zero();
    if (dict) hipLaunchKernelGGL((k_tall_estimate<true>), dim3(grid_for(ncell, kBlock)), dim3(kBlock), 0, st, ncell, cellptr.p, est.p);
    else hipLaunchKernelGGL((k_tall_estimate<false>), dim3(grid_for(ncell, kBlock)), dim3(kBlock), 0, st, ncell, cellptr.p, est.p);
    SLP_HIP(hipGetLastError());
    unsigned long long hest[2];
    est.download(hest, 2);
    static std::atomic<double> last_needs[2][2];
    std::atomic<double> &last_need_slot = last_needs[transposed ? 1 : 0][dict ? 1 : 0];
    const double last_need = last_need_slot.load();
    const double room = (last_need > 0.5 && last_need < 2.0) ? last_need * 1.003 : 1.10;
    i64 cap_w = (i64)((double)hest[0] * room) + 65536, cap_p = 2 * (i64)hest[1] + 4096;
    if (const char *e = getenv("SLP_TALL_BUILD_ROOM")) cap_w = std::max<i64>(4, (i64)((double)hest[0] * atof(e)));
    i64 tot_w = 0, tot_p = 0;
    DevBuf<i64> ext(4 * (size_t)V);
    std::vector<i64> hext(4 * (size_t)V);
    DevBuf<unsigned int> spay, sdir;
    DevBuf<double> spayv;
    for (int attempt = 0;; ++attempt) {
        spay.release();
        spayv.release();
        spay.alloc((size_t)cap_w + 64);
        sdir.alloc((size_t)cap_p * 8);
        if (!dict) spayv.alloc((size_t)cap_w + 64);
        SLP_HIP(hipMemsetAsync(scan.p, 0, (2 * (size_t)ncell + 1) * sizeof(unsigned long long), st));
        const unsigned grid = (unsigned)std::min<i64>(ncell, (i64)ctx().num_cu);
        if (dict) hipLaunchKernelGGL((k_tall_build<true>), dim3(grid), dim3(kTallT), 0, st, R, T, S, Cw, sum0, ncell, sorted.p, (const double *)nullptr, cellptr.p, sc,
                                     cap_w, cap_p, reinterpret_cast<TallPkt *>(sdir.p), spay.p, (double *)nullptr);
        else hipLaunchKernelGGL((k_tall_build<false>), dim3(grid), dim3(kTallT), 0, st, R, T, S, Cw, sum0, ncell, sorted.p, svals.p, cellptr.p, sc,
                                cap_w, cap_p, reinterpret_cast<TallPkt *>(sdir.p), spay.p, spayv.p);
        hipLaunchKernelGGL(k_tall_streams, dim3(grid_for(V, kBlock)), dim3(kBlock), 0, st, V, T, S, cellptr.p, sc, ext.p);
        SLP_HIP(hipGetLastError());
        ext.download(hext.data(), hext.size());
        tot_w = hext[4 * (V - 1)] + hext[4 * (V - 1) + 1];
        tot_p = hext[4 * (V - 1) + 2] + hext[4 * (V - 1) + 3];
        if (tot_w <= cap_w && tot_p <= cap_p) break;
        SLP_REQUIRE(attempt == 0, "tall_build: the pass with the exact sizes did not fit");
        cap_w = tot_w; cap_p = tot_p;
    }
    sorted.release();
    svals.release();
    std::vector<i64> hbase((size_t)V + 1), hpkt((size_t)V + 1);
    const i64 limit = dict ? ((i64)1 << 28) : ((i64)1 << 27);
    hpkt[0] = 0;
    for (i64 v = 0; v < V; ++v) {
        if (hext[4 * v + 1] >= limit) return false;
        hbase[v] = hext[4 * v];
        const i64 np = 1 + hext[4 * v + 3];
        hpkt[v + 1] = hpkt[v] + (np + 2 * kTallDepth - 1) / (2 * kTallDepth) * (2 * kTallDepth) + 2 * kTallDepth;
    }
    hbase[V] = tot_w;
    DevBuf<i64> dpkt;
    dpkt.upload(hpkt.data(), hpkt.size());
    if (hest[0]) last_need_slot.store((double)tot_w / (double)hest[0]);
    if (cap_w > tot_w + tot_w / 100 + 65536) {
        DevBuf<unsigned int> exact((size_t)tot_w + 64);
        SLP_HIP(hipMemcpyAsync(exact.p, spay.p, (size_t)tot_w * sizeof(unsigned int), hipMemcpyDeviceToDevice, st));
        DevBuf<double> exactv;
        if (!dict) {
            exactv.alloc((size_t)tot_w + 64);
            SLP_HIP(hipMemcpyAsync(exactv.p, spayv.p, (size_t)tot_w * sizeof(double), hipMemcpyDeviceToDevice, st));
        }
        SLP_HIP(hipStreamSynchronize(st));
        spay = std::move(exact);
        spayv = std::move(exactv);
    }
    f.tall_dir.emplace_back((size_t)hpkt[V] * 8);
    f.tall_pay.emplace_back(std::move(spay));
    DevBuf<unsigned int> &dir = f.tall_dir.back(), &pay = f.tall_pay.back();
    double *vals = nullptr;
    if (!dict) { f.tall_val.emplace_back(std::move(spayv)); vals = f.tall_val.back().p; }
    hipLaunchKernelGGL(k_tall_dir, dim3(grid_for(std::max<i64>(ncell, V), kBlock)), dim3(kBlock), 0, st, ncell, V, T, S, Cw, cellptr.p, sc, ext.p, dpkt.p,
                       reinterpret_cast<const TallPkt *>(sdir.p), reinterpret_cast<TallPkt *>(dir.p));
    SLP_HIP(hipGetLastError());
    std::vector<TallWg> wg((size_t)V);
    for (i64 v = 0; v < V; ++v) {
        const i64 b = v / S;
        wg[(size_t)v].dir = dir.p + hpkt[v] * 8;
        wg[(size_t)v].pay = pay.p + hbase[v];
        wg[(size_t)v].val = vals ? vals + hbase[v] : nullptr;
        wg[(size_t)v].dict = nullptr;
        wg[(size_t)v].npk = hpkt[v + 1] - hpkt[v];
        wg[(size_t)v].row0 = (v % S) * nrowF + b * (i64)R;
        wg[(size_t)v].x0 = 0;
        wg[(size_t)v].ncol = ncolF;
        wg[(size_t)v].nrows = (int)std::min<i64>(R, nrowF - b * (i64)R);
        wg[(size_t)v].D = dict ? dict->D : 0;
    }
    if (S > 1 && V > 8) {
        const i64 q = V / 8, r = V % 8;
        std::vector<TallWg> placed((size_t)V);
        for (i64 orig = 0; orig < V; ++orig) {
            const i64 xcd = orig % 8;
            const i64 pos = (xcd < r ? xcd * (q + 1) : r * (q + 1) + (xcd - r) * q) + orig / 8;
            const i64 sr = pos / B, b = pos % B;
            placed[(size_t)orig] = wg[(size_t)(b * S + sr)];
        }
        wg.swap(placed);
    }
    f.tall_wg.upload(wg.data(), wg.size());
    SLP_HIP(hipStreamSynchronize(st));
    f.tall_bytes = (dir.n + (size_t)tot_w) * sizeof(unsigned int) + (vals ? (size_t)tot_w * sizeof(double) : 0) + wg.size() * sizeof(TallWg) +
                   (dict ? (size_t)dict->D * sizeof(double) : 0);
    f.nrow = nrowF; f.ncol = ncolF; f.nnz = a.nnz; f.T = T; f.B = B; f.C = (int)Cw; f.rpl = 1;
    f.D = dict ? dict->D : 0;
    f.dict = dict ? dict->values.p : nullptr;
    f.tall = true;
    f.tall_R = R;
    f.tall_dcap = plan.dcap;
    f.tall_total = plan.total;
    f.S = S;
    if (S > 1) f.part.alloc((size_t)S * (size_t)nrowF);
    f.ok = true;
    return true;
}

bool tall_wanted(i64 nrow, i64 ncol, i64 nnz) {
    const char *e = getenv("SLP_TALL");
    if (e && e[0] == '0') return false;
    const char *m = getenv("SLP_STRIP_MIN_NNZ");
    const i64 min_nnz = m ? atoll(m) : 30000000ll;
    if (nnz < min_nnz || nrow <= 0 || ncol <= 0) return false;
    const double per_cell = ((double)nnz / (double)nrow) / (double)((ncol + kTallC - 1) / kTallC);
    return per_cell >= 0.05 && per_cell < 2.5;
}

}
```

pysparselp_amd/csrc/slp_tall_item.h:

```cpp
#pragma once

#if defined(__HIPCC__) || defined(__CUDACC__)
#define SLP_ITEM_FN __host__ __device__ constexpr inline
#else
#define SLP_ITEM_FN constexpr inline
#endif

namespace slp {

constexpr int kTallIdBits = 11, kTallColBits = 12, kTallRowBits = 14;
constexpr int kTallItemIdShift = 3, kTallItemColShift = kTallItemIdShift + kTallIdBits;
constexpr int kTallItemSumLoShift = kTallItemColShift + kTallColBits;
constexpr int kTallItemSumLoBits = 32 - kTallItemSumLoShift;
constexpr int kTallItemSumShift = kTallItemSumLoShift - 3;
constexpr unsigned int kTallItemSumMask = ((1u << kTallRowBits) - 1u) << 3;
constexpr unsigned int kTallItemValMask = ((1u << kTallIdBits) - 1u) << kTallItemIdShift;
constexpr unsigned int kTallItemTableByte = 8;
constexpr int kTallItem64SumShift = 3, kTallItem64ColShift = kTallItem64SumShift + kTallRowBits;
static_assert(kTallItemSumLoBits + 8 == kTallRowBits, "the sum field: 6 bits in the word, 8 in the fifth byte");
static_assert(kTallItem64ColShift + kTallColBits <= 32, "fp64 item: sum field and column in one word");

struct TallItem {
    unsigned int word;
    unsigned int fifth;
};

SLP_ITEM_FN unsigned int tall_item_sum_base(int dcap) { return 1u + (unsigned int)dcap; }

SLP_ITEM_FN TallItem tall_item_encode(unsigned int id, unsigned int col, unsigned int sum) {
    return TallItem{(id << kTallItemIdShift) | (col << kTallItemColShift) | ((sum & ((1u << kTallItemSumLoBits) - 1u)) << kTallItemSumLoShift),
                    sum >> kTallItemSumLoBits};
}
SLP_ITEM_FN unsigned int tall_item_sum_bytes(unsigned int word, unsigned int fifth) {
    return ((word >> kTallItemSumShift) | (fifth << (32 - kTallItemSumShift))) & kTallItemSumMask;
}
SLP_ITEM_FN unsigned int tall_item_value_bytes(unsigned int word) { return word & kTallItemValMask; }
SLP_ITEM_FN unsigned int tall_item_column(unsigned int word) { return (word >> kTallItemColShift) & ((1u << kTallColBits) - 1u); }

SLP_ITEM_FN unsigned int tall_item_sum(unsigned int word, unsigned int fifth) { return tall_item_sum_bytes(word, fifth) >> 3; }
SLP_ITEM_FN unsigned int tall_item_id(unsigned int word) { return tall_item_value_bytes(word) >> 3; }

SLP_ITEM_FN unsigned int tall_item64_encode(unsigned int col, unsigned int sum) {
    return (sum << kTallItem64SumShift) | (col << kTallItem64ColShift);
}
SLP_ITEM_FN unsigned int tall_item64_sum_bytes(unsigned int word) { return word & kTallItemSumMask; }
SLP_ITEM_FN unsigned int tall_item64_column(unsigned int word) { return word >> kTallItem64ColShift; }
SLP_ITEM_FN unsigned int tall_item64_sum(unsigned int word) { return tall_item64_sum_bytes(word) >> 3; }

}
```

pysparselp_amd/csrc/slp_tall_plan.h:

```cpp
#pragma once
#include <algorithm>
#include <cmath>
#include <cstdint>

namespace slp {

constexpr int kTallLdsBytes = 160 * 1024;
constexpr int kTallPlanLanes = 1024;
constexpr int kTallDictMax = 2048;
constexpr int kTallCmax = 4096, kTallCmin = 1024, kTallCstep = 256;
constexpr int kTallBuildFixed = 29440;
constexpr int kTallBuildRowBytes = 10;
constexpr int kTallRmax = 13312;
constexpr int kTallRmaxSplit = 9984;
static_assert(kTallBuildFixed + kTallBuildRowBytes * kTallRmax <= kTallLdsBytes && kTallRmax + 1 < (1 << 14), "tall cells: row blocks");
constexpr double kTallListMax = 3.91;

struct TallPlanIn {
    int64_t nrow = 0, ncol = 0, nnz = 0;
    int D = 0;
    int64_t cus = 1;
    int64_t block_multiple = 0;
    int64_t rows_before = 0, rows_total = 0;
    int env_R = 0, env_C = 0, env_split = 0;
    int carry_C = 0, carry_dcap = -1, carry_R = 0;
    int64_t carry_total = 0;
    int64_t carry_blocks = 0;
};

struct TallPlan {
    int R = 0, C = 0, S = 1, dcap = 0;
    int64_t T = 0;
    int64_t total = 0;
    int off_dv = 0, off_xt = 0, lds_bytes = 0;
    int build_lds_bytes = 0;
};

inline int tall_table_capacity(int D) { return D <= 0 ? 0 : std::min(kTallDictMax, (D + 63) / 64 * 64); }
inline int tall_sums_bytes(int R) { return ((R + 1) * 8 + 15) & ~15; }
inline int tall_lds_rows(int C, int dcap) { return (((kTallLdsBytes - 8 * dcap - 16 * C) / 8) & ~1) - 1; }
inline void tall_plan_layout(TallPlan &p) {
    p.off_dv = tall_sums_bytes(p.R);
    p.off_xt = p.off_dv + 8 * p.dcap;
    p.lds_bytes = p.off_xt + 16 * p.C;
    p.build_lds_bytes = kTallBuildFixed + kTallBuildRowBytes * p.R;
}
inline int64_t tall_rows_for_lanes(double per_cell, int64_t cap) {
    const double p2 = 1.0 - std::exp(-per_cell) * (1.0 + per_cell);
    return p2 > 0.0 ? std::min<int64_t>(cap, (int64_t)(900.0 / p2)) : cap;
}

inline void tall_plan_split_geometry(const TallPlanIn &in, int64_t T, double per_cell, int *R_out, int *S_out) {
    const int64_t cus = in.block_multiple > 0 ? std::min<int64_t>(in.block_multiple, in.cus) : in.cus;
    const int64_t rcap = std::max<int64_t>(1024, tall_rows_for_lanes(per_cell, kTallRmaxSplit));
    if (in.env_R <= 0) {
        const int64_t R = std::min<int64_t>(rcap, std::max<int64_t>(in.nrow, 1)), B = (in.nrow + R - 1) / R;
        int64_t S = in.env_split > 0 ? in.env_split : std::max<int64_t>(1, cus / B);
        S = std::max<int64_t>(1, std::min<int64_t>(S, std::max<int64_t>(1, T / 64)));
        if (S > 1) { *R_out = (int)R; *S_out = (int)S; return; }
    }
    *S_out = 1;
    if (in.env_R > 0) { *R_out = std::min(in.env_R, kTallRmaxSplit); return; }
    int64_t k = (in.nrow + cus * rcap - 1) / (cus * rcap);
    if (k < 1) k = 1;
    int64_t R = (in.nrow + k * cus - 1) / (k * cus);
    if (R < 1024) R = std::min<int64_t>(1024, std::max<int64_t>(in.nrow, 1));
    *R_out = (int)std::min<int64_t>(R, rcap);
}

inline double tall_plan_cost(int64_t nrow, int R, int C, double per_cell, bool dict) {
    const double n = std::max(1.0, (double)std::min<int64_t>(R, nrow) * per_cell), tau = std::ceil(n / kTallPlanLanes);
    const double bytes = dict ? 4.0 + 4.0 * std::min(n, (double)kTallPlanLanes) * std::ceil(tau / 4.0) / n : 12.0;
    return 0.393 * bytes + (0.95 + 0.34 * (double)C / kTallCmax) * 4000.0 / n;
}
inline bool tall_plan_admits(int64_t nrow, int R, int C, double per_cell) {
    if (C == 4096 || C == 2048 || C == 1024) return true;
    return (double)std::min<int64_t>(R, nrow) * per_cell / kTallPlanLanes <= kTallListMax;
}

inline bool tall_width_ok(int c) { return c >= kTallCmin && c <= kTallCmax && c % kTallCstep == 0; }

inline int tall_plan_rows(const TallPlanIn &in, int C, int dcap, double per_cell, int64_t *total_out, int64_t *rcap_out) {
    *total_out = 0;
    const int64_t hard = std::min<int64_t>(tall_lds_rows(C, dcap), kTallRmax);
    const int64_t rcap = std::max<int64_t>(1024, tall_rows_for_lanes(per_cell, hard));
    *rcap_out = rcap;
    if (in.env_R > 0) return (int)std::min<int64_t>(in.env_R, hard);
    if (in.carry_R > 0 && in.carry_R <= hard) return in.carry_R;
    if (in.rows_total > 0 && in.rows_before >= 0 && in.rows_before + in.nrow <= in.rows_total && in.env_split == 0) {
        int64_t total = in.carry_total;
        if (total <= 0) {
            int64_t k = std::max<int64_t>(1, (in.rows_total + in.cus * rcap - 1) / (in.cus * rcap));
            for (int tries = 0; tries < 2; ++tries, ++k) {
                const double h = (double)in.rows_total / (double)(k * in.cus);
                if (tries == 1 || ((double)in.nrow > h && h / (1.0 - h / (double)in.nrow) + 1.0 <= (double)rcap)) break;
            }
            total = k * in.cus;
        }
        auto upto = [&](int64_t r) { return (int64_t)((__int128)total * r / in.rows_total); };
        const int64_t before = in.carry_total > 0 ? in.carry_blocks : upto(in.rows_before);
        const int64_t blocks = std::max<int64_t>({upto(in.rows_before + in.nrow) - before, (in.nrow + rcap - 1) / rcap, 1});
        const int64_t R = (in.nrow + blocks - 1) / blocks;
        if (R >= 1024) { *total_out = total; return (int)R; }
    }
    const int64_t cus = in.block_multiple > 0 ? std::min<int64_t>(in.block_multiple, in.cus) : in.cus;
    int64_t k = (in.nrow + cus * rcap - 1) / (cus * rcap);
    if (k < 1) k = 1;
    int64_t R = (in.nrow + k * cus - 1) / (k * cus);
    if (R < 1024) R = std::min<int64_t>(1024, std::max<int64_t>(in.nrow, 1));
    return (int)std::min<int64_t>(R, rcap);
}

inline TallPlan tall_plan(const TallPlanIn &in) {
    TallPlan best;
    const bool dict = in.D > 0;
    const double per_row = (double)in.nnz / (double)std::max<int64_t>(in.nrow, 1);
    if (in.env_split != 0) {
        int C = kTallCmax;
        double bc = 0.0;
        for (int c = kTallCmax; c >= kTallCmin; c /= 2) {
            const int64_t T = (in.ncol + c - 1) / c;
            int R = 0, S = 1;
            tall_plan_split_geometry(in, T, per_row / (double)T, &R, &S);
            const double cost = tall_plan_cost(in.nrow, R, c, per_row / (double)T, dict);
            if (c == kTallCmax || cost < bc) { bc = cost; C = c; }
        }
        if (in.env_C == 4096 || in.env_C == 2048 || in.env_C == 1024) C = in.env_C;
        const int64_t T = (in.ncol + C - 1) / C;
        int R = 0, S = 1;
        tall_plan_split_geometry(in, T, per_row / (double)T, &R, &S);
        if (S > 1) {
            best.R = R; best.C = C; best.S = S; best.T = T; best.dcap = dict ? kTallDictMax : 0;
            tall_plan_layout(best);
            return best;
        }
    }
    int dcap = tall_table_capacity(in.D);
    if (dict && in.carry_dcap >= 0) dcap = in.D <= in.carry_dcap ? in.carry_dcap : kTallDictMax;
    const int forced = in.carry_C > 0 && tall_width_ok(in.carry_C) ? in.carry_C : (tall_width_ok(in.env_C) ? in.env_C : 0);
    double bc = 0.0;
    int keep = 0;
    for (int c = kTallCmax; c >= kTallCmin; c -= kTallCstep) {
        if (forced && c != forced) continue;
        const int64_t T = (in.ncol + c - 1) / c;
        const double pc = per_row / (double)T;
        int64_t total = 0, rcap = 0;
        const int R = tall_plan_rows(in, c, dcap, pc, &total, &rcap);
        if (!forced && !tall_plan_admits(in.nrow, R, c, pc)) continue;
        const double cost = tall_plan_cost(in.nrow, R, c, pc, dict);
        if (best.C == 0 || cost < bc) {
            bc = cost;
            best.R = R; best.C = c; best.S = 1; best.T = T; best.total = total; best.dcap = dcap;
            keep = in.env_R > 0 || (in.rows_total == 0 && in.block_multiple == 0) ? R : (int)rcap;
        }
    }
    if (dict && in.carry_dcap < 0) {
        const int room = (kTallLdsBytes - tall_sums_bytes(std::max(keep, best.R)) - 16 * best.C) / 8;
        best.dcap = std::min(kTallDictMax, std::max(best.dcap, room / 64 * 64));
    }
    tall_plan_layout(best);
    return best;
}

}
```

pysparselp_amd/csrc/slp_tall_spmv.hip:

```cpp
#include <cmath>
#include <cstdlib>
#include <cstring>
#include <vector>

#include "slp_common.h"
#include "slp_kernels.h"
#include "slp_tall.h"

namespace slp {


template <bool DICT>
struct TallRegs {
    unsigned int lo[kTallSlots];
    unsigned int hi[DICT ? 2 : 1];
    double val[DICT ? 1 : kTallSlots];
    double x[4];
};

template <bool DICT, bool ACC, bool POW = false, int CT = 0>
__global__ __launch_bounds__(kTallT) void k_tall_spmv(int nseg, const TallWg *__restrict__ wgs, const double *__restrict__ dict_arg,
                                                      const double *__restrict__ x, double *__restrict__ out, double pw, const int cw,
                                                      const int dcap, const int oxt) {
    const int C = CT ? CT : cw;
    constexpr int kDepth = DICT ? kTallDepth : 2;
    extern __shared__ __attribute__((aligned(16))) double tall_lds[];
    double *const dv = tall_lds + kTallItemTableByte / 8;
    double *const acc = tall_lds + tall_item_sum_base(dcap);
    double *const xt = tall_lds + oxt;
    typedef __attribute__((address_space(3))) double lds_double;
    auto lds_at = [](unsigned int a) -> lds_double & { return *(lds_double *)(unsigned long long)a; };
    const unsigned int lds0 = (unsigned int)(unsigned long long)(lds_double *)tall_lds;
    if (lds0 != 0u) __builtin_trap();
    const unsigned int xtb = 8u * (unsigned int)oxt;
    const int p = threadIdx.x;
    const unsigned int wbase = (unsigned int)__builtin_amdgcn_readfirstlane(p & ~(kWave - 1));
    const bool piece0 = (int)wbase < (C >> 1), piece1 = (int)wbase + kTallT < (C >> 1);
    const int v = blockIdx.x;
    int cur = 0;
    TallWg wg = wgs[v];
    if (p == 0) tall_lds[0] = 0.0;
    for (int r = p; r < wg.nrows; r += kTallT) acc[r] = ACC ? out[wg.row0 + r] : 0.0;
  for (int seg = 0; seg < nseg; ++seg) {
    if (seg > 0) wg = wgs[(i64)seg * gridDim.x + v];
    if (DICT) {
        const double *__restrict__ dsrc = dict_arg ? dict_arg : wg.dict;
        for (int q = p; q < wg.D; q += kTallT) dv[q] = dsrc[q];
    }
    typedef const unsigned int __attribute__((address_space(1))) *gptr_t;
    const gptr_t hd = (gptr_t)(unsigned long long)wg.dir + (p & 7);
    const int npk = (int)wg.npk - 2 * kTallDepth;
    const __amdgpu_buffer_rsrc_t rs_x =
        __builtin_amdgcn_make_buffer_rsrc(const_cast<double *>(x + wg.x0), 0, (int)(wg.ncol * 8), 0x00020000);

    typedef unsigned int rsrc_words_t __attribute__((ext_vector_type(4)));
    auto words_of = [](const void *base) {
        const unsigned long long a = (unsigned long long)base;
        rsrc_words_t d;
        d[0] = (unsigned int)a; d[1] = (unsigned int)(a >> 32) & 0xffffu; d[2] = 0u; d[3] = 0x00020000u;
        return d;
    };
    auto as_rsrc = [](const rsrc_words_t &d) {
        __amdgpu_buffer_rsrc_t r;
        __builtin_memcpy(&r, &d, sizeof(r));
        return r;
    };
    rsrc_words_t dpay = words_of(wg.pay), dval = words_of(DICT ? (const void *)x : (const void *)wg.val);
    auto slot_pay = [&](unsigned int end) { dpay[2] = end; return as_rsrc(dpay); };
    auto slot_val = [&](unsigned int end) { dval[2] = 2u * end; return as_rsrc(dval); };

    TallRegs<DICT> regs[kDepth];
    unsigned int hw[kDepth];

    struct TallHdr {
        unsigned int off;
        unsigned int xw;
        unsigned int w[kTallSlots];
    };
    static_assert(kTallT <= (1 << 14), "a width's two bits below its upper half-word are zero: (c >> 14) is 4 x the upper width");
    auto unpack = [&](unsigned int h) {
        TallHdr t;
        t.off = (unsigned int)__builtin_amdgcn_readlane((int)h, 0) * 4u;
        t.xw = (unsigned int)__builtin_amdgcn_readlane((int)h, 1);
#pragma unroll
        for (int i = 0; i < 4; ++i) {
            const unsigned int v = (unsigned int)__builtin_amdgcn_readlane((int)h, 2 + i);
            t.w[2 * i] = (v & 0xffffu) * 4u;
            t.w[2 * i + 1] = v >> 14;
        }
        return t;
    };
    const unsigned int wbytes = wbase * 4u;
    unsigned int xwq[kDepth], c4q[kDepth];

    auto load_tile = [&](TallRegs<DICT> &g, const unsigned int xo) {
#pragma unroll
        for (int i = 0; i < 2; ++i) {
            const unsigned int o = (i == 0 ? piece0 : piece1) && xo != kOob ? xo + (unsigned int)i * (unsigned int)(kTallT * 16) : kOob;
            const auto v = __builtin_amdgcn_raw_buffer_load_b128(rs_x, o, 0, 0);
            g.x[2 * i] = __hiloint2double((int)v[1], (int)v[0]);
            g.x[2 * i + 1] = __hiloint2double((int)v[3], (int)v[2]);
        }
    };

    auto issue_part = [&](TallRegs<DICT> &g, const TallHdr &t, const int part) {
        const unsigned int mine = (unsigned int)p * 4u;
        if (part == 0 || wbytes < t.w[4]) {
            unsigned int so = t.off;
            if (part == 1) so += t.w[0] + t.w[1] + t.w[2] + t.w[3];
#pragma unroll
            for (int k = 4 * part; k < 4 * part + 4; ++k) {
                const unsigned int end = so + t.w[k];
                g.lo[k] = __builtin_amdgcn_raw_buffer_load_b32(slot_pay(end), mine, (int)so, 2);
                if (!DICT) {
                    const auto v = __builtin_amdgcn_raw_buffer_load_b64(slot_val(end), 2u * mine, (int)(2u * so), 2);
                    g.val[DICT ? 0 : k] = __hiloint2double((int)v[1], (int)v[0]);
                }
                so = end;
            }
            if (DICT) {
                if (part == 0) so += t.w[4] + t.w[5] + t.w[6] + t.w[7];
                else so += t.w[0];
                g.hi[DICT ? part : 0] = __builtin_amdgcn_raw_buffer_load_b32(slot_pay(so + t.w[4 * part]), mine, (int)so, 2);
            }
        }
        if (part == 1) {
            const unsigned int xs = t.xw & 0x7fffffffu;
            const unsigned int xo = xs == kNoTile ? kOob : (xs + 2u * (unsigned int)p) * 8u;
            load_tile(g, xo);
        }
    };

    auto consume = [&](TallRegs<DICT> &g, const unsigned int xw, const unsigned int c4, auto &&between) {
        if (xw & kPktNewCell) {
            asm volatile("s_waitcnt lgkmcnt(0)\n\ts_barrier" ::: "memory");
            cur = C - cur;
        }
        auto stage_tile = [&]() {
            if ((xw & 0x7fffffffu) != kNoTile) {
                double *dst = static_cast<double *>(__builtin_assume_aligned(xt + (C - cur) + 2 * p, 16));
                if (piece0) *reinterpret_cast<double2 *>(dst) = make_double2(g.x[0], g.x[1]);
                if (piece1) *reinterpret_cast<double2 *>(dst + 2 * kTallT) = make_double2(g.x[2], g.x[3]);
            }
        };
        stage_tile();
        const unsigned int tileb = xtb + 8u * (unsigned int)cur;
        auto group = [&](const int k0) {
            unsigned int w[4], sa[4];
            double ar[4], pr[4], t[4];
#pragma unroll
            for (int k = 0; k < 4; ++k) {
                w[k] = g.lo[k0 + k];
                sa[k] = (DICT ? tall_item_sum_bytes(w[k], g.hi[DICT ? (k0 >> 2) : 0] >> (8 * k)) : tall_item64_sum_bytes(w[k]));
            }
#pragma unroll
            for (int k = 0; k < 4; ++k) ar[k] = lds_at(sa[k]);
#pragma unroll
            for (int k = 0; k < 4; ++k) {
                unsigned int col = DICT ? tall_item_column(w[k]) : tall_item64_column(w[k]);
                asm("" : "+v"(col));
                const double xv = lds_at((col << 3) + tileb);
                pr[k] = DICT ? lds_at(tall_item_value_bytes(w[k]) + kTallItemTableByte) * xv
                             : (POW ? abs_pow(g.val[DICT ? 0 : k0 + k], pw) * 1.0 : g.val[DICT ? 0 : k0 + k]) * xv;
            }
            t[0] = ar[0] + pr[0];
#pragma unroll
            for (int k = 1; k < 4; ++k) t[k] = ((sa[k] == sa[k - 1]) ? t[k - 1] : ar[k]) + pr[k];
#pragma unroll
            for (int k = 0; k < 4; ++k) lds_at(sa[k]) = t[k];
        };
        group(0);
        between();
        if (wbytes < c4) group(4);
    };

#pragma unroll
    for (int u = 0; u < kDepth; ++u) {
        const TallHdr t = unpack(hd[(i64)u * 8]);
        xwq[u] = t.xw;
        c4q[u] = t.w[4];
        issue_part(regs[u], t, 0);
        issue_part(regs[u], t, 1);
        hw[u] = hd[(i64)(u + kDepth) * 8];
    }
    __syncthreads();
    for (int jj = 0; jj < npk; jj += 2 * kDepth) {
#pragma unroll
        for (int u = 0; u < 2 * kDepth; ++u) {
            const int i = u % kDepth;
            const unsigned int xw = xwq[i], c4 = c4q[i];
            TallHdr t;
            consume(regs[i], xw, c4, [&]() {
                t = unpack(hw[i]);
                xwq[i] = t.xw;
                c4q[i] = t.w[4];
                issue_part(regs[i], t, 0);
            });
            issue_part(regs[i], t, 1);
            hw[i] = hd[(i64)(jj + u + 2 * kDepth) * 8];
        }
    }
    __syncthreads();
  }
    for (int r = p; r < wg.nrows; r += kTallT) out[wg.row0 + r] = acc[r];
}


__global__ void k_tall_combine(i64 nrow, int S, const double *__restrict__ part, double *__restrict__ out, int accum) {
    for (i64 r = (i64)blockIdx.x * blockDim.x + threadIdx.x; r < nrow; r += (i64)gridDim.x * blockDim.x) {
        double a = accum ? out[r] + part[r] : part[r];
        for (int s = 1; s < S; ++s) a += part[(i64)s * nrow + r];
        out[r] = a;
    }
}

template <bool DICT, bool ACC, bool POW>
static void tall_launch(const StripJds &f, unsigned grid, int nseg, const TallWg *wgs, const double *dict, const double *x, double *out, double pw) {
    TallPlan lay;
    lay.R = f.tall_R; lay.C = (int)f.C; lay.dcap = DICT ? f.tall_dcap : 0;
    tall_plan_layout(lay);
    SLP_REQUIRE(tall_width_ok(lay.C) && lay.R > 0 && lay.lds_bytes <= kTallLdsBytes && f.D <= lay.dcap, "tall cells: LDS layout");
    auto go = [&](auto kernel, bool &raised) {
        if (!raised) {
            SLP_HIP(hipFuncSetAttribute(reinterpret_cast<const void *>(kernel), hipFuncAttributeMaxDynamicSharedMemorySize, kTallLdsBytes));
            raised = true;
        }
        hipLaunchKernelGGL(kernel, dim3(grid), dim3(kTallT), (size_t)lay.lds_bytes, ctx().stream, nseg, wgs, dict, x, out, pw, lay.C, lay.dcap,
                           lay.off_xt / 8);
    };
    static bool raised[3] = {false, false, false};
    if (DICT && !POW && lay.C == 3072) go(k_tall_spmv<DICT, ACC, POW, (DICT && !POW) ? 3072 : 0>, raised[1]);
    else if (DICT && !POW && lay.C == 4096) go(k_tall_spmv<DICT, ACC, POW, (DICT && !POW) ? 4096 : 0>, raised[2]);
    else go(k_tall_spmv<DICT, ACC, POW, 0>, raised[0]);
}

void tall_spmv(const StripJds &f, const double *x, double *out, int accum) {
    double *dst = f.S > 1 ? f.part.p : out;
    const unsigned grid = (unsigned)(f.B * f.S);
    const bool acc = accum && f.S == 1;
    const double *none = nullptr;
    if (f.D > 0) { if (acc) tall_launch<true, true, false>(f, grid, 1, f.tall_wg.p, f.dict, x, dst, 0.0); else tall_launch<true, false, false>(f, grid, 1, f.tall_wg.p, f.dict, x, dst, 0.0); }
    else { if (acc) tall_launch<false, true, false>(f, grid, 1, f.tall_wg.p, none, x, dst, 0.0); else tall_launch<false, false, false>(f, grid, 1, f.tall_wg.p, none, x, dst, 0.0); }
    if (f.S > 1)
        hipLaunchKernelGGL(k_tall_combine, dim3(grid_for(f.nrow, kBlock)), dim3(kBlock), 0, ctx().stream, f.nrow, f.S, f.part.p, out, accum);
    SLP_HIP(hipGetLastError());
}

void tall_spmv_fused(const StripJds &f, const double *x, double *out) {
    const int nseg = f.parts_cols ? (int)f.parts.size() : 1;
    const unsigned grid = (unsigned)(f.tall_wg.n / (size_t)nseg);
    if (f.D > 0) tall_launch<true, false, false>(f, grid, nseg, f.tall_wg.p, nullptr, x, out, 0.0);
    else tall_launch<false, false, false>(f, grid, nseg, f.tall_wg.p, nullptr, x, out, 0.0);
    SLP_HIP(hipGetLastError());
}

bool tall_fuse(StripJds &f) {
    f.tall_wg.release();
    const char *e = getenv("SLP_TALL_FUSE");
    if (e && e[0] == '0') return false;
    if (f.parts.empty()) return false;
    const StripJds &f0 = *f.parts[0];
    for (const StripJds *g : f.parts)
        if (!g->ok || !g->tall || g->S != 1 || g->C != f0.C || (g->D > 0) != (f0.D > 0) || g->tall_dcap != f0.tall_dcap ||
            (f.parts_cols && (g->B != f0.B || g->tall_R != f0.tall_R || g->nrow != f0.nrow)))
            return false;
    std::vector<TallWg> all;
    for (size_t k = 0; k < f.parts.size(); ++k) {
        const StripJds &g = *f.parts[k];
        std::vector<TallWg> wg((size_t)g.B);
        SLP_HIP(hipMemcpy(wg.data(), g.tall_wg.p, wg.size() * sizeof(TallWg), hipMemcpyDeviceToHost));
        for (TallWg &w : wg) {
            w.dict = g.dict;
            if (f.parts_cols) w.x0 = f.part_off[k];
            else w.row0 += f.part_off[k];
            all.push_back(w);
        }
    }
    f.tall_wg.upload(all.data(), all.size());
    f.C = f0.C;
    f.tall_dcap = f0.tall_dcap;
    f.tall_R = 0;
    for (const StripJds *g : f.parts) f.tall_R = std::max(f.tall_R, g->tall_R);
    return true;
}

void tall_spmv_pow(const StripJds &f, double pw, const double *x, double *out, int accum) {
    SLP_REQUIRE(f.ok && f.tall && f.D == 0, "tall_spmv_pow: not a tall-cell copy with fp64 entries");
    double *dst = f.S > 1 ? f.part.p : out;
    const unsigned grid = (unsigned)(f.B * f.S);
    if (accum && f.S == 1) tall_launch<false, true, true>(f, grid, 1, f.tall_wg.p, nullptr, x, dst, pw);
    else tall_launch<false, false, true>(f, grid, 1, f.tall_wg.p, nullptr, x, dst, pw);
    if (f.S > 1)
        hipLaunchKernelGGL(k_tall_combine, dim3(grid_for(f.nrow, kBlock)), dim3(kBlock), 0, ctx().stream, f.nrow, f.S, f.part.p, out, accum);
    SLP_HIP(hipGetLastError());
}
}
```

Before: 11.73.

## Interleave first four tall-packet slots into per-lane records for 128-bit loads

Adds a 'records' packet layout for the tall-cell SpMV, in which the first four item slots of each lane are stored contiguously so the kernel can fetch them with one 128-bit buffer load instead of four separate 32-bit loads. The builder, size estimator, planner and SpMV kernel gain a REC template parameter. By default the layout is chosen only for dictionary-encoded matrices whose padding growth stays under 1/16, and chunks share the choice through the carry. The cost is extra padding words and more kernel instantiations.

Result: faster. 12.00 (median of 6 runs) (+2.3%).

```diff
diff --git a/include/slp_hip_ext.h b/include/slp_hip_ext.h
--- a/include/slp_hip_ext.h
+++ b/include/slp_hip_ext.h
@@ -6,6 +6,7 @@
 #include "slp_hip.h"
 #include "slp_hip_ext_admm_batch.h"
 #include "slp_hip_ext_dga_batch.h"
+#include "slp_hip_ext_tall.h"
 
 #ifdef __cplusplus
 extern "C" {
diff --git a/include/slp_hip_ext_tall.h b/include/slp_hip_ext_tall.h
--- /dev/null
+++ b/include/slp_hip_ext_tall.h
@@ -0,0 +1,17 @@
+#ifndef SLP_HIP_EXT_TALL_H
+#define SLP_HIP_EXT_TALL_H
+
+#include <stdint.h>
+
+#include "slp_hip.h"
+
+#ifdef __cplusplus
+extern "C" {
+#endif
+
+int64_t slp_matrix_tall_records(slp_matrix *a, int transposed);
+
+#ifdef __cplusplus
+}
+#endif
+#endif
diff --git a/pysparselp_amd/_lib.py b/pysparselp_amd/_lib.py
--- a/pysparselp_amd/_lib.py
+++ b/pysparselp_amd/_lib.py
@@ -263,6 +263,12 @@
 
 EXT_DGA_BATCH_SYMBOLS = tuple(_EXT_DGA_BATCH_SIGNATURES)
 
+_EXT_TALL_SIGNATURES = {
+    "slp_matrix_tall_records": (c_i64, [c_vp, c_int]),
+}
+
+EXT_TALL_SYMBOLS = tuple(_EXT_TALL_SIGNATURES)
+
 HOST_ALLREDUCE_FN = ctypes.CFUNCTYPE(c_int, ctypes.POINTER(c_dbl), c_i64, c_int, c_vp)
 
 
@@ -284,7 +290,7 @@
     except OSError as e:
         raise SlpError(f"cannot load {LIB_PATH}: {e}") from e
     for name, (res, args) in (list(_SIGNATURES.items()) + list(_EXT_SIGNATURES.items()) + list(_EXT_ADMM_BATCH_SIGNATURES.items())
-                              + list(_EXT_DGA_BATCH_SIGNATURES.items())):
+                              + list(_EXT_DGA_BATCH_SIGNATURES.items()) + list(_EXT_TALL_SIGNATURES.items())):
         fn = getattr(lib, name)
         fn.restype = res
         fn.argtypes = args
diff --git a/pysparselp_amd/csrc/slp_chunked.hip b/pysparselp_amd/csrc/slp_chunked.hip
--- a/pysparselp_amd/csrc/slp_chunked.hip
+++ b/pysparselp_amd/csrc/slp_chunked.hip
@@ -1,5 +1,6 @@
 #include "slp_common.h"
 #include "slp_kernels.h"
+#include "../../include/slp_hip_ext_tall.h"
 
 slp_matrix::~slp_matrix() {
     for (slp_matrix *c : chunks) delete c;
@@ -97,6 +98,7 @@
                 if (f->tall && f->S == 1) {
                     g->tall_carry[t].C = f->C; g->tall_carry[t].dcap = f->D > 0 ? f->tall_dcap : -1;
                     g->tall_carry[t].R = f->tall_R; g->tall_carry[t].total = f->tall_total;
+                    g->tall_carry[t].records = f->tall_records ? 1 : 0;
                 }
             }
         if (f0->tall) g->tall_carry[0].blocks += f0->B;
@@ -162,6 +164,19 @@
     return rc == 0 ? r : -1;
 }
 
+int64_t slp_matrix_tall_records(slp_matrix *m, int transposed) {
+    if (!m) return -1;
+    int64_t r = 0;
+    const int rc = [&]() -> int {
+        SLP_API_INT({
+            const StripJds *f = fast_format(m, transposed != 0);
+            if (f && !m->chunks.empty() && !f->parts.empty()) f = f->parts[0];
+            r = (f && f->ok && f->tall && f->tall_records) ? 1 : 0;
+        })
+    }();
+    return rc == 0 ? r : -1;
+}
+
 int64_t slp_matrix_product_launches(const slp_matrix *g, int transposed) {
     if (!g) return -1;
     if (g->chunks.empty()) return 1;
diff --git a/pysparselp_amd/csrc/slp_common.h b/pysparselp_amd/csrc/slp_common.h
--- a/pysparselp_amd/csrc/slp_common.h
+++ b/pysparselp_amd/csrc/slp_common.h
@@ -230,6 +230,7 @@
     bool tall = false;
     int tall_R = 0;
     int tall_dcap = 0;
+    bool tall_records = false;
     i64 tall_total = 0;
     DevBuf<TallWg> tall_wg;
     std::vector<DevBuf<unsigned int>> tall_dir;
@@ -263,6 +264,7 @@
 bool tall_wanted(i64 nrow, i64 ncol, i64 nnz);
 struct TallCarry {
     int C = 0, dcap = -1, R = 0;
+    int records = -1;
     i64 total = 0;
     i64 blocks = 0;
 };
diff --git a/pysparselp_amd/csrc/slp_tall.hip b/pysparselp_amd/csrc/slp_tall.hip
--- a/pysparselp_amd/csrc/slp_tall.hip
+++ b/pysparselp_amd/csrc/slp_tall.hip
@@ -161,7 +161,7 @@
     return s;
 }
 
-template <bool DICT>
+template <bool DICT, bool REC>
 __global__ __launch_bounds__(kTallT) void k_tall_build(int R, i64 T, int S, int C, unsigned int sum0, i64 ncell, const unsigned long long *__restrict__ keys,
                                                        const double *__restrict__ svals, const i64 *__restrict__ cellptr, TallScan sc,
                                                        i64 cap_w, i64 cap_p, TallPkt *__restrict__ sdir,
@@ -425,8 +425,7 @@
         nlane[p] = cover;
         unsigned long long cw = 0;
         {
-            unsigned long long w = cover;
-            if (DICT) w += (cover + 7u) / 8u + (cover > 4u ? (cover - 4u + 7u) / 8u : 0u);
+            unsigned long long w = tall_packet_lane_words(cover, DICT, REC);
             w = tall_lane_sums<kWave>(w);
             if ((p & (kWave - 1)) == kWave - 1) wtot[p / kWave] = w;
         }
@@ -453,10 +452,10 @@
             }
             __syncthreads();
             SLP_TB_PROF(8);
-            unsigned int wd[kTallSlots], words = 0;
-            for (int j = 0; j < kTallSlots; ++j) { wd[j] = width[j]; words += wd[j]; }
-            const unsigned int hi0 = words, hi1 = words + wd[0];
-            if (DICT) words += wd[0] + wd[4];
+            unsigned int wd[kTallSlots];
+            for (int j = 0; j < kTallSlots; ++j) wd[j] = width[j];
+            const TallPacketLayout lay = tall_packet_layout(wd, DICT, REC);
+            const unsigned int words = lay.words;
             unsigned int kofs[kTallSlots], have = 0;
 #pragma unroll
             for (int j = 0; j < kTallSlots; ++j) {
@@ -521,10 +520,10 @@
             if (!fits) break;
             {
                 unsigned int *base = pay + woff;
-                unsigned int hb0 = 0, hb1 = 0, so = 0;
+                unsigned int hb0 = 0, hb1 = 0;
 #pragma unroll
                 for (int j = 0; j < kTallSlots; ++j) {
-                    if ((unsigned)p < wd[j]) {
+                    if ((unsigned)p < wd[REC && j < 4 ? 0 : j]) {
                         unsigned int item = 0u, hib = 0u;
                         if (have >> j & 1u) {
                             const unsigned int r1 = ((unsigned int)(key[j] >> (kTallIdBits + kTallColBits)) & ((1u << kTallRowBits) - 1)) + sum0;
@@ -537,15 +536,15 @@
                                 item = tall_item64_encode(cl, r1);
                             }
                         }
-                        base[so + p] = item;
-                        if (!DICT) payv[woff + so + p] = value[j];
+                        const unsigned int at = tall_packet_item_word(lay, REC, (unsigned)p, j);
+                        base[at] = item;
+                        if (!DICT) payv[woff + at] = value[j];
                         if (j < 4) hb0 |= hib << (8 * j);
                         else hb1 |= hib << (8 * (j - 4));
                     }
-                    so += wd[j];
                 }
-                if (DICT && (unsigned)p < wd[0]) base[hi0 + p] = hb0;
-                if (DICT && (unsigned)p < wd[4]) base[hi1 + p] = hb1;
+                if (DICT && (unsigned)p < wd[0]) base[lay.fifth0 + p] = hb0;
+                if (DICT && (unsigned)p < wd[4]) base[lay.fifth1 + p] = hb1;
                 if (p == 0) {
                     TallPkt h;
                     h.off = woff;
@@ -565,14 +564,14 @@
 }
 
 template <bool DICT>
-__global__ __launch_bounds__(kBlock) void k_tall_estimate(i64 ncell, const i64 *__restrict__ cellptr, unsigned long long *__restrict__ est) {
+__global__ __launch_bounds__(kBlock) void k_tall_estimate(i64 ncell, const i64 *__restrict__ cellptr, int records, unsigned long long *__restrict__ est) {
     unsigned long long w = 0, k = 0;
     for (i64 c = (i64)blockIdx.x * kBlock + threadIdx.x; c < ncell; c += (i64)gridDim.x * kBlock) {
         const unsigned long long n = (unsigned long long)(cellptr[c + 1] - cellptr[c]);
         if (!n) continue;
         const unsigned long long L = n < (unsigned)kTallT ? n : (unsigned)kTallT, tau = (n + kTallT - 1) / kTallT;
-        unsigned long long cw = n;
-        if (DICT) cw += L * ((tau + 7) / 8 + (tau > 4 ? (tau - 4 + 7) / 8 : 0));
+        const unsigned long long cw = records ? tall_packet_balanced_words(n, kTallT, DICT, true)
+                                              : n + L * (tall_packet_lane_words((unsigned int)tau, DICT, false) - tau);
         w += (cw + 3ull) & ~3ull;
         k += (tau + kTallSlots - 1) / kTallSlots;
     }
@@ -650,7 +649,9 @@
     pin.nrow = nrowF; pin.ncol = ncolF; pin.nnz = a.nnz; pin.D = dict ? dict->D : 0; pin.cus = ctx().num_cu;
     if (!transposed) { pin.block_multiple = block_multiple; pin.rows_before = rows_before; pin.rows_total = rows_total; }
     pin.env_R = std::max(0, tall_env("SLP_TALL_R")); pin.env_C = tall_env("SLP_TALL_C"); pin.env_split = tall_env("SLP_TALL_SPLIT");
+    if (const char *e = getenv("SLP_TALL_RECORDS")) pin.env_records = atoi(e) != 0 ? 1 : 0;
     if (carry && carry->C > 0) {
+        pin.carry_records = carry->records;
         pin.carry_C = carry->C; pin.carry_dcap = carry->dcap; pin.carry_total = transposed ? 0 : carry->total;
         pin.carry_R = transposed ? carry->R : 0;
         pin.carry_blocks = transposed ? 0 : carry->blocks;
@@ -659,6 +660,7 @@
     SLP_REQUIRE(plan.lds_bytes <= kTallLdsBytes && plan.build_lds_bytes <= kTallLdsBytes && plan.R >= 1 && plan.R <= kTallRmax,
                 "tall_build: the planned geometry does not fit the LDS");
     const int R = plan.R, S = plan.S, Cw = plan.C;
+    const bool records = plan.records;
     const i64 T = plan.T;
     const unsigned int sum0 = tall_item_sum_base(plan.dcap);
     SLP_REQUIRE(sum0 + (unsigned int)R <= (1u << kTallRowBits), "tall_build: sum field");
@@ -749,13 +751,13 @@
     TallScan sc;
     sc.w = scan.p; sc.p = scan.p + ncell; sc.ticket = scan.p + 2 * ncell; sc.before_w = sc.ticket + 1; sc.before_p = sc.before_w + ncell;
     est.zero();
-    if (dict) hipLaunchKernelGGL((k_tall_estimate<true>), dim3(grid_for(ncell, kBlock)), dim3(kBlock), 0, st, ncell, cellptr.p, est.p);
-    else hipLaunchKernelGGL((k_tall_estimate<false>), dim3(grid_for(ncell, kBlock)), dim3(kBlock), 0, st, ncell, cellptr.p, est.p);
+    if (dict) hipLaunchKernelGGL((k_tall_estimate<true>), dim3(grid_for(ncell, kBlock)), dim3(kBlock), 0, st, ncell, cellptr.p, records ? 1 : 0, est.p);
+    else hipLaunchKernelGGL((k_tall_estimate<false>), dim3(grid_for(ncell, kBlock)), dim3(kBlock), 0, st, ncell, cellptr.p, records ? 1 : 0, est.p);
     SLP_HIP(hipGetLastError());
     unsigned long long hest[2];
     est.download(hest, 2);
-    static std::atomic<double> last_needs[2][2];
-    std::atomic<double> &last_need_slot = last_needs[transposed ? 1 : 0][dict ? 1 : 0];
+    static std::atomic<double> last_needs[2][2][2];
+    std::atomic<double> &last_need_slot = last_needs[transposed ? 1 : 0][dict ? 1 : 0][records ? 1 : 0];
     const double last_need = last_need_slot.load();
     const double room = (last_need > 0.5 && last_need < 2.0) ? last_need * 1.003 : 1.10;
     i64 cap_w = (i64)((double)hest[0] * room) + 65536, cap_p = 2 * (i64)hest[1] + 4096;
@@ -773,10 +775,12 @@
         if (!dict) spayv.alloc((size_t)cap_w + 64);
         SLP_HIP(hipMemsetAsync(scan.p, 0, (2 * (size_t)ncell + 1) * sizeof(unsigned long long), st));
         const unsigned grid = (unsigned)std::min<i64>(ncell, (i64)ctx().num_cu);
-        if (dict) hipLaunchKernelGGL((k_tall_build<true>), dim3(grid), dim3(kTallT), 0, st, R, T, S, Cw, sum0, ncell, sorted.p, (const double *)nullptr, cellptr.p, sc,
-                                     cap_w, cap_p, reinterpret_cast<TallPkt *>(sdir.p), spay.p, (double *)nullptr);
-        else hipLaunchKernelGGL((k_tall_build<false>), dim3(grid), dim3(kTallT), 0, st, R, T, S, Cw, sum0, ncell, sorted.p, svals.p, cellptr.p, sc,
-                                cap_w, cap_p, reinterpret_cast<TallPkt *>(sdir.p), spay.p, spayv.p);
+        auto build = [&](auto kernel) {
+            hipLaunchKernelGGL(kernel, dim3(grid), dim3(kTallT), 0, st, R, T, S, Cw, sum0, ncell, sorted.p, dict ? (const double *)nullptr : svals.p, cellptr.p, sc,
+                               cap_w, cap_p, reinterpret_cast<TallPkt *>(sdir.p), spay.p, dict ? (double *)nullptr : spayv.p);
+        };
+        if (dict) { if (records) build(k_tall_build<true, true>); else build(k_tall_build<true, false>); }
+        else { if (records) build(k_tall_build<false, true>); else build(k_tall_build<false, false>); }
         hipLaunchKernelGGL(k_tall_streams, dim3(grid_for(V, kBlock)), dim3(kBlock), 0, st, V, T, S, cellptr.p, sc, ext.p);
         SLP_HIP(hipGetLastError());
         ext.download(hext.data(), hext.size());
@@ -856,6 +860,7 @@
     f.tall = true;
     f.tall_R = R;
     f.tall_dcap = plan.dcap;
+    f.tall_records = records;
     f.tall_total = plan.total;
     f.S = S;
     if (S > 1) f.part.alloc((size_t)S * (size_t)nrowF);
diff --git a/pysparselp_amd/csrc/slp_tall_item.h b/pysparselp_amd/csrc/slp_tall_item.h
--- a/pysparselp_amd/csrc/slp_tall_item.h
+++ b/pysparselp_amd/csrc/slp_tall_item.h
@@ -47,4 +47,47 @@
 SLP_ITEM_FN unsigned int tall_item64_column(unsigned int word) { return word >> kTallItem64ColShift; }
 SLP_ITEM_FN unsigned int tall_item64_sum(unsigned int word) { return tall_item64_sum_bytes(word) >> 3; }
 
+struct TallPacketLayout {
+    unsigned int slot[8];
+    unsigned int fifth0;
+    unsigned int fifth1;
+    unsigned int words;
+};
+SLP_ITEM_FN unsigned int tall_packet_record_word(unsigned int lane, int slot) { return 4u * lane + (unsigned int)slot; }
+SLP_ITEM_FN unsigned int tall_packet_group1_word(const unsigned int *w, bool dict, bool records) {
+    return records ? (dict ? 5u : 4u) * w[0] : w[0] + w[1] + w[2] + w[3];
 }
+SLP_ITEM_FN TallPacketLayout tall_packet_layout(const unsigned int *w, bool dict, bool records) {
+    TallPacketLayout l{};
+    unsigned int so = 0;
+    for (int k = 0; k < 4; ++k) { l.slot[k] = so; so += records ? 0u : w[k]; }
+    so = tall_packet_group1_word(w, dict, records);
+    for (int k = 4; k < 8; ++k) { l.slot[k] = so; so += w[k]; }
+    if (records) {
+        l.fifth0 = 4u * w[0];
+        l.fifth1 = so;
+        l.words = so + (dict ? w[4] : 0u);
+    } else {
+        l.fifth0 = so;
+        l.fifth1 = so + w[0];
+        l.words = so + (dict ? w[0] + w[4] : 0u);
+    }
+    return l;
+}
+SLP_ITEM_FN unsigned int tall_packet_item_word(const TallPacketLayout &l, bool records, unsigned int lane, int k) {
+    return records && k < 4 ? tall_packet_record_word(lane, k) : l.slot[k] + lane;
+}
+SLP_ITEM_FN unsigned int tall_packet_lane_words(unsigned int len, bool dict, bool records) {
+    const unsigned int n0 = (len + 7u) / 8u;
+    const unsigned int n1 = len > 4u ? (len + 3u) / 8u : 0u;
+    if (!records) return len + (dict ? n0 + n1 : 0u);
+    const unsigned int second = 4u * (len / 8u) + (len % 8u > 4u ? len % 8u - 4u : 0u);
+    return 4u * n0 + second + (dict ? n0 + n1 : 0u);
+}
+SLP_ITEM_FN unsigned long long tall_packet_balanced_words(unsigned long long n, unsigned int lanes, bool dict, bool records) {
+    if (!n) return 0ull;
+    const unsigned long long tau = (n + lanes - 1u) / lanes, more = n % lanes ? n % lanes : lanes;
+    return more * tall_packet_lane_words((unsigned int)tau, dict, records) + (lanes - more) * tall_packet_lane_words((unsigned int)tau - 1u, dict, records);
+}
+
+}
diff --git a/pysparselp_amd/csrc/slp_tall_plan.h b/pysparselp_amd/csrc/slp_tall_plan.h
--- a/pysparselp_amd/csrc/slp_tall_plan.h
+++ b/pysparselp_amd/csrc/slp_tall_plan.h
@@ -2,6 +2,8 @@
 #include <algorithm>
 #include <cmath>
 #include <cstdint>
+
+#include "slp_tall_item.h"
 
 namespace slp {
 
@@ -26,10 +28,13 @@
     int carry_C = 0, carry_dcap = -1, carry_R = 0;
     int64_t carry_total = 0;
     int64_t carry_blocks = 0;
+    int env_records = -1;
+    int carry_records = -1;
 };
 
 struct TallPlan {
     int R = 0, C = 0, S = 1, dcap = 0;
+    bool records = false;
     int64_t T = 0;
     int64_t total = 0;
     int off_dv = 0, off_xt = 0, lds_bytes = 0;
@@ -76,6 +81,20 @@
 inline bool tall_plan_admits(int64_t nrow, int R, int C, double per_cell) {
     if (C == 4096 || C == 2048 || C == 1024) return true;
     return (double)std::min<int64_t>(R, nrow) * per_cell / kTallPlanLanes <= kTallListMax;
+}
+
+constexpr double kTallRecordGrowth = 1.0 / 16;
+inline int64_t tall_plan_cell_items(int64_t nrow, int R, double per_cell) {
+    return std::max<int64_t>(1, std::llround((double)std::min<int64_t>(R, nrow) * per_cell));
+}
+inline double tall_plan_record_growth(int64_t nrow, int R, double per_cell, bool dict) {
+    const uint64_t n = (uint64_t)tall_plan_cell_items(nrow, R, per_cell);
+    return (double)tall_packet_balanced_words(n, kTallPlanLanes, dict, true) / (double)tall_packet_balanced_words(n, kTallPlanLanes, dict, false) - 1.0;
+}
+inline bool tall_plan_records(const TallPlanIn &in, int R, double per_cell, bool dict) {
+    if (in.env_records >= 0) return in.env_records != 0;
+    if (in.carry_records >= 0 && dict == (in.carry_dcap >= 0)) return in.carry_records != 0;
+    return dict && tall_plan_record_growth(in.nrow, R, per_cell, dict) <= kTallRecordGrowth;
 }
 
 inline bool tall_width_ok(int c) { return c >= kTallCmin && c <= kTallCmax && c % kTallCstep == 0; }
@@ -131,6 +150,7 @@
         tall_plan_split_geometry(in, T, per_row / (double)T, &R, &S);
         if (S > 1) {
             best.R = R; best.C = C; best.S = S; best.T = T; best.dcap = dict ? kTallDictMax : 0;
+            best.records = tall_plan_records(in, R, per_row / (double)T, dict);
             tall_plan_layout(best);
             return best;
         }
@@ -158,6 +178,7 @@
         const int room = (kTallLdsBytes - tall_sums_bytes(std::max(keep, best.R)) - 16 * best.C) / 8;
         best.dcap = std::min(kTallDictMax, std::max(best.dcap, room / 64 * 64));
     }
+    best.records = tall_plan_records(in, best.R, per_row / (double)best.T, dict);
     tall_plan_layout(best);
     return best;
 }
diff --git a/pysparselp_amd/csrc/slp_tall_spmv.hip b/pysparselp_amd/csrc/slp_tall_spmv.hip
--- a/pysparselp_amd/csrc/slp_tall_spmv.hip
+++ b/pysparselp_amd/csrc/slp_tall_spmv.hip
@@ -1,6 +1,7 @@
 #include <cmath>
 #include <cstdlib>
 #include <cstring>
+#include <type_traits>
 #include <vector>
 
 #include "slp_common.h"
@@ -18,7 +19,7 @@
     double x[4];
 };
 
-template <bool DICT, bool ACC, bool POW = false, int CT = 0>
+template <bool DICT, bool ACC, bool POW = false, int CT = 0, bool REC = false>
 __global__ __launch_bounds__(kTallT) void k_tall_spmv(int nseg, const TallWg *__restrict__ wgs, const double *__restrict__ dict_arg,
                                                       const double *__restrict__ x, double *__restrict__ out, double pw, const int cw,
                                                       const int dcap, const int oxt) {
@@ -105,9 +106,23 @@
 
     auto issue_part = [&](TallRegs<DICT> &g, const TallHdr &t, const int part) {
         const unsigned int mine = (unsigned int)p * 4u;
-        if (part == 0 || wbytes < t.w[4]) {
+        if (REC && part == 0) {
+            const unsigned int so = t.off, end = so + 4u * t.w[0];
+            const auto v = __builtin_amdgcn_raw_buffer_load_b128(slot_pay(end), 4u * mine, (int)so, 2);
+#pragma unroll
+            for (int k = 0; k < 4; ++k) g.lo[k] = v[k];
+            if (!DICT) {
+#pragma unroll
+                for (int h = 0; h < 2; ++h) {
+                    const auto u = __builtin_amdgcn_raw_buffer_load_b128(slot_val(end), 8u * mine + 16u * (unsigned int)h, (int)(2u * so), 2);
+                    g.val[DICT ? 0 : 2 * h] = __hiloint2double((int)u[1], (int)u[0]);
+                    g.val[DICT ? 0 : 2 * h + 1] = __hiloint2double((int)u[3], (int)u[2]);
+                }
+            }
+            if (DICT) g.hi[0] = __builtin_amdgcn_raw_buffer_load_b32(slot_pay(end + t.w[0]), mine, (int)end, 2);
+        } else if (part == 0 || wbytes < t.w[4]) {
             unsigned int so = t.off;
-            if (part == 1) so += t.w[0] + t.w[1] + t.w[2] + t.w[3];
+            if (part == 1) so += tall_packet_group1_word(t.w, DICT, REC);
 #pragma unroll
             for (int k = 4 * part; k < 4 * part + 4; ++k) {
                 const unsigned int end = so + t.w[k];
@@ -120,7 +135,7 @@
             }
             if (DICT) {
                 if (part == 0) so += t.w[4] + t.w[5] + t.w[6] + t.w[7];
-                else so += t.w[0];
+                else if (!REC) so += t.w[0];
                 g.hi[DICT ? part : 0] = __builtin_amdgcn_raw_buffer_load_b32(slot_pay(so + t.w[4 * part]), mine, (int)so, 2);
             }
         }
@@ -228,10 +243,15 @@
         hipLaunchKernelGGL(kernel, dim3(grid), dim3(kTallT), (size_t)lay.lds_bytes, ctx().stream, nseg, wgs, dict, x, out, pw, lay.C, lay.dcap,
                            lay.off_xt / 8);
     };
-    static bool raised[3] = {false, false, false};
-    if (DICT && !POW && lay.C == 3072) go(k_tall_spmv<DICT, ACC, POW, (DICT && !POW) ? 3072 : 0>, raised[1]);
-    else if (DICT && !POW && lay.C == 4096) go(k_tall_spmv<DICT, ACC, POW, (DICT && !POW) ? 4096 : 0>, raised[2]);
-    else go(k_tall_spmv<DICT, ACC, POW, 0>, raised[0]);
+    static bool raised[2][3] = {{false, false, false}, {false, false, false}};
+    auto by_width = [&](auto rec) {
+        constexpr bool REC = decltype(rec)::value;
+        if (DICT && !POW && lay.C == 3072) go(k_tall_spmv<DICT, ACC, POW, (DICT && !POW) ? 3072 : 0, REC>, raised[REC][1]);
+        else if (DICT && !POW && lay.C == 4096) go(k_tall_spmv<DICT, ACC, POW, (DICT && !POW) ? 4096 : 0, REC>, raised[REC][2]);
+        else go(k_tall_spmv<DICT, ACC, POW, 0, REC>, raised[REC][0]);
+    };
+    if (f.tall_records) by_width(std::true_type());
+    else by_width(std::false_type());
 }
 
 void tall_spmv(const StripJds &f, const double *x, double *out, int accum) {
@@ -262,6 +282,7 @@
     const StripJds &f0 = *f.parts[0];
     for (const StripJds *g : f.parts)
         if (!g->ok || !g->tall || g->S != 1 || g->C != f0.C || (g->D > 0) != (f0.D > 0) || g->tall_dcap != f0.tall_dcap ||
+            g->tall_records != f0.tall_records ||
             (f.parts_cols && (g->B != f0.B || g->tall_R != f0.tall_R || g->nrow != f0.nrow)))
             return false;
     std::vector<TallWg> all;
@@ -279,6 +300,7 @@
     f.tall_wg.upload(all.data(), all.size());
     f.C = f0.C;
     f.tall_dcap = f0.tall_dcap;
+    f.tall_records = f0.tall_records;
     f.tall_R = 0;
     for (const StripJds *g : f.parts) f.tall_R = std::max(f.tall_R, g->tall_R);
     return true;
```
